# yjtang249/MIPSFusion

Measured on AMD Instinct MI355X. Metric: rays*samples/s per GPU, full optimisation iteration (fwd + bwd + pose+map Adam), 4096 rays x 64 samples, 640x480 RGB-D, higher is better.
Workload: dtype f32; decoder products as 3 x bf16 pieces of each fp32 operand, 6 bf16 MFMAs per product, fp32 accumulate; 1 GPU; BASELINE config 2: FastCaMo-synth apartment_2, 1 active submap per GPU, 4096 rays x 64 samples, hash grid 2^19 x 16 x 2, 620x460 synthetic RGB-D; rays=4096, samples_per_ray=64, hash_size=19, parallelism=single gpu

## Files before the change

### include/mipsf_compact.h

```cpp
#ifndef MIPSF_COMPACT_H
#define MIPSF_COMPACT_H

#include "mipsf.h"

#ifdef __cplusplus
extern "C" {
#endif

#define MIPSF_LIVE_HEADER 16u
#define MIPSF_LIVE_PAD 0xffffffffu
int mipsf_decoder_live_compact(const float* dout, uint32_t M, uint32_t* live_list, float* dfeat, float* dx, int feat_layout,
                               void* stream);

int mipsf_hashgrid_dx_from_jac_list(const float* jac, const float* dout, float* dx, const uint32_t* live_list, uint32_t M,
                                    const mipsf_grid_meta* meta_host, int layout, void* stream);

int mipsf_gather_pose_place_fwd_masked(const float* db, uint64_t n_rows, const int64_t* idx, const float* fixed_poses,
                                       const float* rot, const float* trans, uint32_t F, uint32_t K, const int64_t* owner,
                                       const float* noise, const float* z_uniform, const float* z_near_offsets,
                                       const float* z_near_nodepth, const mipsf_render_cfg* cfg_host, float* d_cam, float* rgb,
                                       float* depth, float* z_vals, float* xn, uint32_t* counts, uint32_t* wants_dx, uint32_t N,
                                       void* stream);
int mipsf_hashgrid_fwd_masked(const float* x, const float* params, float* out, float* jac, const uint32_t* ray_mask, uint32_t S,
                              uint32_t M, const mipsf_grid_meta* meta_host, int layout, void* stream);
int mipsf_hashgrid_dx_from_jac_masked(const float* jac, const float* dout, float* dx, const uint32_t* tile_live,
                                      const uint32_t* live_list, const uint32_t* ray_mask, uint32_t S, uint32_t M,
                                      const mipsf_grid_meta* meta_host, int layout, void* stream);

#ifdef __cplusplus
}
#endif
#endif
```

### mipsfusion_amd/_lib.py

```python
from __future__ import annotations

import ctypes as C
import os
from typing import Optional

import torch

_HERE = os.path.dirname(os.path.abspath(__file__))
LIB_PATH = os.environ.get("MIPSF_LIB") or os.path.join(_HERE, "libmipsf_hip.so")
MAX_LEVELS = 32
FEAT_AOS, FEAT_LEVEL_MAJOR = 0, 1
PREC = {"f32": 0, "f16x3": 1, "f16": 2, "bf16x3": 3, "bf16x6": 4}


class GridMeta(C.Structure):
    _fields_ = [("n_levels", C.c_uint32), ("n_features", C.c_uint32), ("log2_hashmap_size", C.c_uint32),
                ("base_resolution", C.c_uint32), ("per_level_scale", C.c_float),
                ("log2_per_level_scale", C.c_float), ("n_params", C.c_uint32),
                ("offsets", C.c_uint32 * (MAX_LEVELS + 1)), ("resolutions", C.c_uint32 * MAX_LEVELS),
                ("scales", C.c_float * MAX_LEVELS)]


class DecoderWeights(C.Structure):
    _fields_ = [(n, C.c_void_p) for n in ("w_pts0", "b_pts0", "w_pts2", "b_pts2", "w_rgb0", "b_rgb0",
# ... 65 lines not shown


class AdamTensors(C.Structure):
    _fields_ = [("count", C.c_uint32), ("param", C.c_void_p * ADAM_MAX_TENSORS), ("grad", C.c_void_p * ADAM_MAX_TENSORS),
                ("exp_avg", C.c_void_p * ADAM_MAX_TENSORS), ("exp_avg_sq", C.c_void_p * ADAM_MAX_TENSORS),
                ("numel", C.c_uint64 * ADAM_MAX_TENSORS)]


ADAM_MAX_GROUPS = 8
ADAM_SMALL_MAX_NUMEL = 16384


class AdamSmall(C.Structure):
    _fields_ = [("n_groups", C.c_uint32), ("n_tensors", C.c_uint32),
                ("step_dev", C.c_void_p * ADAM_MAX_GROUPS), ("hyper_dev", C.c_void_p * ADAM_MAX_GROUPS),
                ("lr", C.c_float * ADAM_MAX_GROUPS), ("beta1", C.c_float * ADAM_MAX_GROUPS),
                ("beta2", C.c_float * ADAM_MAX_GROUPS), ("eps", C.c_float * ADAM_MAX_GROUPS),
                ("weight_decay", C.c_float * ADAM_MAX_GROUPS),
                ("param", C.c_void_p * ADAM_MAX_TENSORS), ("grad", C.c_void_p * ADAM_MAX_TENSORS),
                ("exp_avg", C.c_void_p * ADAM_MAX_TENSORS), ("exp_avg_sq", C.c_void_p * ADAM_MAX_TENSORS),
                ("numel", C.c_uint32 * ADAM_MAX_TENSORS), ("group_of", C.c_uint32 * ADAM_MAX_TENSORS)]


_P = C.c_void_p
_U32, _U64, _I, _F, _D = C.c_uint32, C.c_uint64, C.c_int, C.c_float, C.c_double

SIGNATURES = {
    "mipsf_last_error": (C.c_char_p, []),
    "mipsf_abi_version": (_I, []),
    "mipsf_device_cu_count": (_I, []),
    "mipsf_buffer_size": (_U64, [_I, _U32, _U32, _U32, C.POINTER(GridMeta)]),
    "mipsf_hashgrid_meta_init": (_I, [C.POINTER(GridMeta), _U32, _U32, _U32, _U32, _D]),
    "mipsf_hashgrid_fwd": (_I, [_P, _P, _P, _P, _U32, C.POINTER(GridMeta), _I, _P]),
    "mipsf_hashgrid_dx_from_jac": (_I, [_P, _P, _P, _P, _U32, C.POINTER(GridMeta), _I, _P]),
    "mipsf_hashgrid_bwd": (_I, [C.POINTER(HashgridBwdArgs), _P]),
    "mipsf_hashgrid_route": (_I, [_P, _P, _U32, C.POINTER(GridMeta), _P]),    "mipsf_hashgrid_indices": (_I, [_P, _P, _U32, C.POINTER(GridMeta), _P]),
    "mipsf_freq_fwd": (_I, [_P, _P, _U32, _U32, _U32, _P]),
    "mipsf_freq_bwd": (_I, [_P, _P, _P, _U32, _U32, _U32, _P]),
    "mipsf_decoder_pack": (_I, [C.POINTER(DecoderWeights), _P, _P]),
    "mipsf_decoder_pack_host": (_I, [C.POINTER(DecoderWeights), _P]),
    "mipsf_decoder_fwd": (_I, [_P, _P, _I, _P, _P, _I, _P, _P, _U32, _P]),
    "mipsf_decoder_fwd_sdf": (_I, [_P, _P, _I, _P, _P, _I, _P, _U32, _P]),
    "mipsf_decoder_bwd": (_I, [_P, _P, _I, _P, _P, _I, _P, _P, _P, _P, _P, _P, C.POINTER(DecoderGrads), _P, _P,
                               _U32, _P]),
    "mipsf_decoder_bwd_chain": (_I, [_P, _I, _P, _I, _P, _P, _P, _P, _P, _P, _P, _U32, _P]),
    "mipsf_decoder_wgrad": (_I, [_P, _I, _P, _P, _I, _P, _P, C.POINTER(DecoderGrads), _P, _I, _U32, _P]),
    "mipsf_decoder_pack16": (_I, [C.POINTER(DecoderWeights), _P, _I, _P]),
    "mipsf_decoder_fwd16": (_I, [C.POINTER(DecoderFwd16Args), _P]),
    "mipsf_decoder_bwd_chain16": (_I, [C.POINTER(DecoderChain16Args), _P]),
    "mipsf_decoder_wgrad16": (_I, [C.POINTER(DecoderWgrad16Args), _P]),
    "mipsf_sample_rays": (_I, [_P, _P, _P, _P, _P, _P, _P, C.POINTER(RenderCfg), _P, _P, _P, _U32, _P]),
    "mipsf_normalise_points": (_I, [_P, C.POINTER(RenderCfg), _P, _U32, _P]),
    "mipsf_render_fwd": (_I, [C.POINTER(RenderFwdArgs), _P]),
    "mipsf_loss_finalize_sums": (_I, [_P, C.POINTER(RenderCfg), _U32, _U32, _P, _P, _P, _P]),
    "mipsf_render_bwd": (_I, [C.POINTER(RenderBwdArgs), _P]),
    "mipsf_gather_pose_place_fwd": (_I, [_P, _U64, _P, _P, _P, _P, _U32, _U32, _P, _P, _P, _P, _P, C.POINTER(RenderCfg), _P, _P,
                                         _P, _P, _P, _P, _U32, _P]),
    "mipsf_place_pose_bwd": (_I, [_P, _P, C.POINTER(RenderCfg), _P, _U32, _U32, _P, _P, _P, _P, _P, _U32, _U32, _I, _P]),
    "mipsf_rays_bwd": (_I, [_P, _P, C.POINTER(RenderCfg), _P, _P, _U32, _U32, _P]),
    "mipsf_normalise_bwd": (_I, [_P, C.POINTER(RenderCfg), _P, _U32, _P]),
    "mipsf_pose_rays_fwd": (_I, [_P, _U64, _P, _P, _P, _P, _U32, _U32, _P, _P, _P, _P, _P, _P, _U32, _P]),
    "mipsf_pose_handover": (_I, [_P, _I, _P, _P, _P]),
    "mipsf_pose_rays_bwd": (_I, [_P, _P, _P, _U32, _U32, _P, _P, _P, _P, _P, _U32, _I, _P]),
    "mipsf_adam_step": (_I, [_P, _P, _P, _P, _U64, _F, _F, _F, _F, _F, _U32, _P, _I, _P]),
    "mipsf_adam_advance_n": (_I, [_P, _P, _P, _P, _P, _U32, _P]),
    "mipsf_adam_step_multi": (_I, [C.POINTER(AdamTensors), _F, _F, _F, _F, _F, _U32, _P, _I, _P]),
    "mipsf_adam_step_small": (_I, [C.POINTER(AdamSmall), _I, _P]),
    "mipsf_adam_step_all": (_I, [C.POINTER(AdamSmall), _I, _P, _P]),
    "mipsf_ro_fitness": (_I, [_P, _U32, _P, _F, _P, _U32, _U32, _P]),
    "mipsf_ro_fitness_sdf": (_I, [_P, _P, _F, _P, _U32, _U32, _I, _P]),
    "mipsf_ro_particles": (_I, [_P, _P, _P, _P, C.POINTER(RenderCfg), _P, _P, _U32, _U32, _I, _P]),
    "mipsf_ro_update": (_I, [_P, _P, _P, _F, _F, _U32, _P]),
    "mipsf_gather_rays": (_I, [_P, _U64, _P, _U32, _P, _P, _P, _P, _P]),
}


SIZE_MCUBES_OFFSET_WORDS, SIZE_MCUBES_WELD_SLOTS, SIZE_MCUBES_WELD_WORDS = 20, 21, 22
MCUBES_BLOCK_CELLS = 4096
McubesArgs = _args("McubesArgs", [("X", _CU), ("Y", _CU), ("Z", _CU), ("isovalue", C.c_float), ("truncation", C.c_float),
                                  ("volume", _VP), ("cases", _VP), ("block_offsets", _VP), ("soup", _VP), ("cell_ids", _VP),
                                  ("capacity_tris", _CU)])
McubesWeldArgs = _args("McubesWeldArgs", [("T", _CU), ("soup", _VP), ("scratch", _VP), ("vertices", _VP), ("faces", _VP),
                                          ("counts", _VP), ("max_rounds", _CU)])
COMPACT_SIGNATURES = {
    "mipsf_decoder_live_compact": (_I, [_P, _U32, _P, _P, _P, _I, _P]),
    "mipsf_hashgrid_dx_from_jac_list": (_I, [_P, _P, _P, _P, _U32, C.POINTER(GridMeta), _I, _P]),
    "mipsf_gather_pose_place_fwd_masked": (_I, [_P, _U64, _P, _P, _P, _P, _U32, _U32, _P, _P, _P, _P, _P, C.POINTER(RenderCfg),
                                                _P, _P, _P, _P, _P, _P, _P, _U32, _P]),
    "mipsf_hashgrid_fwd_masked": (_I, [_P, _P, _P, _P, _P, _U32, _U32, C.POINTER(GridMeta), _I, _P]),
    "mipsf_hashgrid_dx_from_jac_masked": (_I, [_P, _P, _P, _P, _P, _P, _U32, _U32, C.POINTER(GridMeta), _I, _P]),
}

MESH_SIGNATURES = {
    "mipsf_mcubes_count": (_I, [C.POINTER(McubesArgs), _P]),
    "mipsf_mcubes_emit": (_I, [C.POINTER(McubesArgs), _P]),
    "mipsf_mcubes_weld": (_I, [C.POINTER(McubesWeldArgs), _P]),
}


FUSE_KF_FLOATS = 16
FUSE_IN_BOX, FUSE_SEEN = 1, 2


class FusePoints(C.Structure):
    _fields_ = [("points", _VP), ("ticks", _VP * 3), ("dims", _CU * 3), ("lo", _CU * 3), ("size", _CU * 3), ("first", _CU), ("n", _CU)]


class FuseCamera(C.Structure):
    _fields_ = [("fx", C.c_float), ("fy", C.c_float), ("cx", C.c_float), ("cy", C.c_float), ("W", C.c_float), ("H", C.c_float),
                ("edge", C.c_float), ("k", _CU), ("keyframes", _VP)]


FuseVisibilityArgs = _args("FuseVisibilityArgs", [("pts", FusePoints), ("cam", FuseCamera), ("seen", _VP)])
FuseLocalArgs = _args("FuseLocalArgs", [("pts", FusePoints), ("w2l", C.c_float * 12), ("sub", C.c_double * 3), ("div", C.c_double * 3),
                                        ("out", _VP)])
FuseAccumulateArgs = _args("FuseAccumulateArgs", [("pts", FusePoints), ("cam", FuseCamera), ("rows", _VP), ("n_rows", _CU),
                                                  ("channels", _CU), ("sigmoid", _CU), ("values", _VP), ("entropy", _VP),
                                                  ("value_stride", _CU), ("entropy_stride", _CU), ("use_obb", _CU),
                                                  ("obb_centre", C.c_double * 3), ("obb_axes", C.c_double * 9),
                                                  ("obb_half", C.c_double * 3), ("centroid", C.c_float * 3), ("sigma", C.c_float),
                                                  ("gauss_k", C.c_float), ("num", _VP), ("den", _VP), ("flags", _VP)])
FuseFinalizeArgs = _args("FuseFinalizeArgs", [("n", _CU), ("channels", _CU), ("num", _VP), ("den", _VP), ("flags", _VP), ("out", _VP),
                                              ("volume", _VP)])
FuseLabelArgs = _args("FuseLabelArgs", [("F", _CU), ("E", _CU), ("pairs", _VP), ("labels", _VP), ("counts", _VP), ("max_rounds", _CU),
                                        ("resume", _CU)])
FUSE_SIGNATURES = {
    "mipsf_fuse_visibility": (_I, [C.POINTER(FuseVisibilityArgs), _P]),
    "mipsf_fuse_local_points": (_I, [C.POINTER(FuseLocalArgs), _P]),
    "mipsf_fuse_accumulate": (_I, [C.POINTER(FuseAccumulateArgs), _P]),
    "mipsf_fuse_finalize": (_I, [C.POINTER(FuseFinalizeArgs), _P]),
    "mipsf_fuse_label_components": (_I, [C.POINTER(FuseLabelArgs), _P]),
}


ICP_KNN = 30
ICP_RESULT_DOUBLES = 20
ICP_MAX_POINTS, ICP_MAX_CELLS = 1 << 27, 1 << 26
ICP_WS_CLOUD, ICP_WS_GRID, ICP_WS_REGISTER = 1, 2, 3
IcpCloudArgs = _args("IcpCloudArgs", [("n", _CU), ("k", _CU), ("rows_per_owner", _CU), ("rows", _VP), ("owner", _VP), ("poses", _VP),
                                      ("points", _VP), ("count", _VP), ("workspace", _VP)])
IcpBinArgs = _args("IcpBinArgs", [("n", _CU), ("max_cells", _CU), ("points", _VP), ("min_edge", C.c_double), ("grid", _VP)])
IcpNearestArgs = _args("IcpNearestArgs", [("n_source", _CU), ("n_target", _CU), ("max_cells", _CU), ("source", _VP), ("grid", _VP),
                                          ("max_dist", C.c_double), ("partner", _VP), ("d2", _VP)])
IcpNormalsArgs = _args("IcpNormalsArgs", [("n", _CU), ("max_cells", _CU), ("points", _VP), ("grid", _VP), ("normals", _VP),
                                          ("neighbours", _VP)])
IcpRegisterArgs = _args("IcpRegisterArgs", [("n_source", _CU), ("n_target", _CU), ("max_cells", _CU), ("max_iteration", _CU),
                                            ("source", _VP), ("grid", _VP), ("target_normals", _VP), ("max_dist", C.c_double),
                                            ("relative_fitness", C.c_double), ("relative_rmse", C.c_double), ("result", _VP),
                                            ("partner", _VP), ("workspace", _VP)])
ICP_SIGNATURES = {
    "mipsf_icp_workspace_bytes": (_U64, [_I, _U32, _U32]),
    "mipsf_icp_cloud": (_I, [C.POINTER(IcpCloudArgs), _P]),
    "mipsf_icp_bin": (_I, [C.POINTER(IcpBinArgs), _P]),
    "mipsf_icp_nearest": (_I, [C.POINTER(IcpNearestArgs), _P]),
    "mipsf_icp_normals": (_I, [C.POINTER(IcpNormalsArgs), _P]),
    "mipsf_icp_register": (_I, [C.POINTER(IcpRegisterArgs), _P]),
}


POSEGRAPH_MAX_NODES, POSEGRAPH_MAX_EDGES, POSEGRAPH_LDS_NODES, POSEGRAPH_RESULT_DOUBLES = 64, 1024, 20, 8
POSEGRAPH_FACTORISATION_FAILED, POSEGRAPH_NAN_QUALITY, POSEGRAPH_BAD_EDGE = 1, 2, 4
PosegraphArgs = _args("PosegraphArgs", [("n_nodes", _CU), ("n_edges", _CU), ("input_f64", _CU), ("anchors", _VP), ("edges", _VP),
                                        ("observations", _VP), ("weights", _VP), ("steps", _CU), ("patience", _CU),
                                        ("max_rejects", _CU), ("reserved", _CU), ("decreasing", C.c_double), ("radius", C.c_double),
                                        ("min_diag", C.c_double), ("anchors_out", _VP), ("anchors_out32", _VP), ("result", _VP),
                                        ("workspace", _VP)])
POSEGRAPH_SIGNATURES = {
# ... 355 lines not shown
```

### mipsfusion_amd/csrc/decoder.hip

```cpp
#include "decoder_dev.h"
#include "launch.h"

namespace mipsf {
using namespace dl;


template <bool PE_INTERNAL, int LAYOUT, bool SAVE, bool SDF_ONLY = false>
__device__ __forceinline__ void decoder_fwd_tile(const float* tail, const float4* img1,
                                                 const float4* img2, const float4* img3,
                                                 const float* __restrict__ feat, const float* __restrict__ x,
                                                 const float* __restrict__ embed_pos, float* __restrict__ out,
                                                 float* __restrict__ saved, uint32_t M, int pin, int64_t tile,
                                                 int lane) {
    const int j = lane & 31, h = lane >> 5;
    const uint32_t s_raw = (uint32_t)(tile * 32 + j);
    const bool live = s_raw < M;
    const uint32_t s = live ? s_raw : M - 1;
    const uint32_t lane16 = 16u * (uint32_t)lane;
    const srd_t sv = make_srd(SAVE ? saved + (size_t)tile * ACT_TILE_FLOATS : saved, SAVE ? ACT_TILE_FLOATS * 4 : 0);

    float ev[E_SLOTS];
    load_e<PE_INTERNAL>(x, embed_pos, s, h, ev);

    f32x16 H1[4];
    load_bias(tail, 0, h, H1);
    mfma_layer<RT_F1, T_F1>(img1, lane, H1,
                            [&](int t) { return t < E_SLOTS ? ev[t] : 0.0f; });
#pragma unroll
    for (int rt = 0; rt < 4; ++rt)
#pragma unroll
        for (int r = 0; r < 16; ++r) H1[rt][r] = fmaxf(H1[rt][r], 0.0f);

    uint32_t m1[2] = {0u, 0u};
    if (SAVE) relu_masks(H1, m1);

    constexpr int RT2 = SDF_ONLY ? 2 : RT_F2;
    f32x16 H2[RT2];
    load_bias(tail, 1, h, H2);
    mfma_layer<RT2, T_F2>(img2, lane, H2,
                          [&](int t) { return H1[t >> 4][t & 15]; },
                          [&](int t4) { if constexpr (SAVE) { if (pin == 0) buf_store_act_piece(sv, lane16, 0, H1, t4); } });

    float rgb[3] = {0.f, 0.f, 0.f};
    if constexpr (!SDF_ONLY) {
        float pr[3];
        const float4* trgb = reinterpret_cast<const float4*>(tail) + h * TRGB_SLOTS;
        f32x2 p01 = {0.f, 0.f};
        float p2 = 0.f;
#pragma unroll
        for (int slot = 0; slot < 32; ++slot) {
            const float4 wv = trgb[slot];
            const float v = H2[2 + (slot >> 4)][slot & 15];
            p01 = __builtin_elementwise_fma(f32x2{wv.x, wv.y}, f32x2{v, v}, p01);
            p2 = fmaf(wv.z, v, p2);
        }
#pragma unroll
        for (int t = 0; t < E_SLOTS; ++t) {
            const float4 wv = trgb[32 + t];
            p01 = __builtin_elementwise_fma(f32x2{wv.x, wv.y}, f32x2{ev[t], ev[t]}, p01);
            p2 = fmaf(wv.z, ev[t], p2);
        }
        pr[0] = p01.x, pr[1] = p01.y, pr[2] = p2;
#pragma unroll
        for (int c = 0; c < 3; ++c) rgb[c] = (pr[c] + __shfl_xor(pr[c], 32, 64)) + tail[OFF_BSMALL - OFF_TRGB + c];
    }

    float gf[16];
    if (LAYOUT == MIPSF_FEAT_LEVEL_MAJOR && M < (1u << 24)) {
        const srd_t fs = make_srd(feat, M * 128u);
        const uint32_t voff = (2u * s + (uint32_t)h) * 4u;
#pragma unroll
        for (int u = 0; u < 16; ++u)
            gf[u] = __uint_as_float(__builtin_amdgcn_raw_buffer_load_b32(fs, voff, (uint32_t)u * M * 8u, 0));
    } else {
#pragma unroll
        for (int u = 0; u < 16; ++u) gf[u] = load_feat<LAYOUT>(feat, s, u, h, M);
    }
    f32x16 H3[4];
    load_bias(tail, 2, h, H3);
    mfma_layer<RT_F3, T_F3>(img3, lane, H3,
                            [&](int t) { return t < 32 ? H2[t >> 4][t & 15] : gf[t - 32]; },
                            [&](int t4) {
                                if constexpr (SAVE) {
// ... 617 lines not shown
        if (!tile_live) zero16(nx);
        put_act(XT, nx, 0, 4, 0, w, lane);
        put_act(YT, ny, 2, 2, 0, w, lane);
        {
            float ev[E_SLOTS];
            load_e<PE_INTERNAL>(x, embed_pos, s, h, ev);
#pragma unroll
            for (int t = 0; t < E_SLOTS; ++t) {
                const int e = eidx(t, h);
                if (e >= 0) YT[e * WG_LDW + 32 * w + j] = ev[t];
            }
        }
        {
            float* pad = YT + (51 + bhalf) * WG_LDW + brow;
#pragma unroll
            for (int i = 0; i < 7; ++i)
                if (bhalf + 2 * i < 13) pad[2 * i * WG_LDW] = (bhalf + 2 * i == 0) ? 1.0f : 0.0f;
        }
        X8[(4 * bhalf + 0) * WG_LDW + brow] = nsm.x;
        X8[(4 * bhalf + 1) * WG_LDW + brow] = nsm.y;
        X8[(4 * bhalf + 2) * WG_LDW + brow] = nsm.z;
        X8[(4 * bhalf + 3) * WG_LDW + brow] = nsm.w;
        __syncthreads();
        {
            const char* by = act_base(saved, tile, 2, 0);
            auto fetch = [&](int g) { ny[g] = act_piece(by, g, lane16); };
            if constexpr (BF16X3) wgrad_mma_bf16<2>(XT, YT, w, 0, lane, aW1, fetch);
            else wgrad_mma<2>(XT, YT, w, 0, lane, aW1, fetch);
        }
        wgrad_mma_small(X8, YT, w, lane, aRGB);
        __syncthreads();

        put_act(YT, ny, 0, 4, 0, w, lane);
        __syncthreads();
        {
            const uint32_t nb = bt + gridDim.x;
            const int nt = src_tile(nb);
            const char* bx = act_base(dact, nt, 2, 0);
            const char* by = act_base(saved, nt, 1, 0);
            const uint32_t ns = sample_of(nb);
            wgrad_mma_small(X8, YT, w, lane, aS2, [&](int g) {
                nx[g] = act_piece(bx, g, lane16);
                if (g < 8) ny[g] = act_piece(by, g, lane16);
                ngf[g] = load_feat<LAYOUT>(feat, ns, g, h, M);
            });
        }
        __syncthreads();
    }

    float* rec = partial + (size_t)blockIdx.x * (G_STRIDE + 0);
    for (int q = tid; q < G_STRIDE; q += DEC_BLOCK) rec[q] = 0.0f;
    __syncthreads();
#pragma unroll
    for (int ct = 0; ct < 3; ++ct) flush_tile(rec, G_W_SDF0, HID, N_SDF_IN, w, ct, lane, aS1[ct]);
#pragma unroll
    for (int ct = 0; ct < 4; ++ct) flush_tile(rec, G_W_PTS2, HID, HID, w, ct, lane, aW2[ct]);
#pragma unroll
    for (int ct = 0; ct < 2; ++ct) flush_tile(rec, G_W_PTS0, HID, N_E, w, ct, lane, aW1[ct]);
    {
#pragma unroll
        for (int ct = 0; ct < 2; ++ct)
#pragma unroll
            for (int r = 0; r < 4; ++r) {
                const int row = 4 * (lane >> 4) + r, col = 32 * w + 16 * ct + (lane & 15);
                if (row < N_CLASS) rec[G_W_SDF2 + row * HID + col] = aS2[ct][r];
                const int rc = col < N_E ? 64 + col : (col >= 64 ? col - 64 : -1);
                if (row >= 5 && row < 8 && rc >= 0) rec[G_W_RGB0 + (row - 5) * N_RGB_IN + rc] = aRGB[ct][r];
                if (col == N_E && row < N_CLASS) rec[G_B_SDF2 + row] = aRGB[ct][r];
                if (col == N_E && row >= 5 && row < 8) rec[G_B_RGB0 + row - 5] = aRGB[ct][r];
            }
    }
    {
        const int jj = lane & 31, hh = lane >> 5;
        if (jj == N_E - 32) {
#pragma unroll
            for (int r = 0; r < 16; ++r) rec[G_B_PTS0 + 32 * w + rowmap(r, hh)] = aW1[1][r];
        }
    }
    atomicAdd(&rec[G_B_SDF0 + brow], db3);
    atomicAdd(&rec[G_B_PTS2 + brow], db2);
}


struct GradPtrs {
    float* p[10];
};

constexpr int WG_REDUCE_SLICES = 8;
__global__ __launch_bounds__(256) void decoder_wgrad_reduce_kernel(const float* __restrict__ partial, uint32_t nrec,
                                                                   GradPtrs g) {
    const int q = blockIdx.x * blockDim.x + threadIdx.x;
    if (q >= G_TOTAL) return;
    float a0 = 0.f, a1 = 0.f, a2 = 0.f, a3 = 0.f;
    uint32_t b = blockIdx.y;
    for (; b + 3 * WG_REDUCE_SLICES < nrec; b += 4 * WG_REDUCE_SLICES) {
        a0 += partial[(size_t)b * G_STRIDE + q];
        a1 += partial[(size_t)(b + WG_REDUCE_SLICES) * G_STRIDE + q];
        a2 += partial[(size_t)(b + 2 * WG_REDUCE_SLICES) * G_STRIDE + q];
        a3 += partial[(size_t)(b + 3 * WG_REDUCE_SLICES) * G_STRIDE + q];
    }
    for (; b < nrec; b += WG_REDUCE_SLICES) a0 += partial[(size_t)b * G_STRIDE + q];
    const float a = (a0 + a1) + (a2 + a3);
    const int bounds[11] = {G_W_PTS0, G_B_PTS0, G_W_PTS2, G_B_PTS2, G_W_RGB0, G_B_RGB0,
                            G_W_SDF0, G_B_SDF0, G_W_SDF2, G_B_SDF2, G_TOTAL};
#pragma unroll
    for (int k = 0; k < 10; ++k)
        if (q >= bounds[k] && q < bounds[k + 1]) unsafeAtomicAdd(&g.p[k][q - bounds[k]], a);
}

__global__ __launch_bounds__(256) void decoder_pack_kernel(W w, float* __restrict__ packed) {
    const int idx = blockIdx.x * blockDim.x + threadIdx.x;
    if (idx < PACKED_FLOATS) packed[idx] = packed_value(w, idx);
}

static W to_w(const mipsf_decoder_weights& s) {
    W w;
    w.w_pts0 = s.w_pts0, w.b_pts0 = s.b_pts0, w.w_pts2 = s.w_pts2, w.b_pts2 = s.b_pts2, w.w_rgb0 = s.w_rgb0;
    w.b_rgb0 = s.b_rgb0, w.w_sdf0 = s.w_sdf0, w.b_sdf0 = s.b_sdf0, w.w_sdf2 = s.w_sdf2, w.b_sdf2 = s.b_sdf2;
    return w;
}

constexpr uint32_t WG_MAX_BLOCKS = 256;

__global__ __launch_bounds__(256) void decoder_wgrad_reduce_fixed_kernel(const float* __restrict__ partial, uint32_t nrec,
                                                                         GradPtrs g) {
    const int q = blockIdx.x * blockDim.x + threadIdx.x;
    if (q >= G_TOTAL) return;
    float a = 0.f;
    for (uint32_t b = 0; b < nrec; ++b) a += partial[(size_t)b * G_STRIDE + q];
    const int bounds[11] = {G_W_PTS0, G_B_PTS0, G_W_PTS2, G_B_PTS2, G_W_RGB0, G_B_RGB0,
                            G_W_SDF0, G_B_SDF0, G_W_SDF2, G_B_SDF2, G_TOTAL};
#pragma unroll
    for (int k = 0; k < 10; ++k)
        if (q >= bounds[k] && q < bounds[k + 1]) {
            float* p = &g.p[k][q - bounds[k]];
            *p = *p + a;
        }
}

int wgrad_reduce_launch(const float* partial, uint32_t nrec, const mipsf_decoder_grads* grads, hipStream_t s, bool fixed_order) {
    if (fixed_order) {
        GradPtrs g;
        g.p[0] = grads->w_pts0, g.p[1] = grads->b_pts0, g.p[2] = grads->w_pts2, g.p[3] = grads->b_pts2;
        g.p[4] = grads->w_rgb0, g.p[5] = grads->b_rgb0, g.p[6] = grads->w_sdf0, g.p[7] = grads->b_sdf0;
        g.p[8] = grads->w_sdf2, g.p[9] = grads->b_sdf2;
        for (int k = 0; k < 10; ++k) MIPSF_REQUIRE(g.p[k] != nullptr, "null gradient pointer %d", k);
        hipLaunchKernelGGL(decoder_wgrad_reduce_fixed_kernel, dim3((G_TOTAL + 255) / 256), dim3(256), 0, s, partial, nrec, g);
        return check_launch("decoder_wgrad_reduce_fixed");
    }
    return wgrad_reduce_launch(partial, nrec, grads, s);
}

int wgrad_reduce_launch(const float* partial, uint32_t nrec, const mipsf_decoder_grads* grads, hipStream_t s) {
    GradPtrs g;
    g.p[0] = grads->w_pts0, g.p[1] = grads->b_pts0, g.p[2] = grads->w_pts2, g.p[3] = grads->b_pts2;
    g.p[4] = grads->w_rgb0, g.p[5] = grads->b_rgb0, g.p[6] = grads->w_sdf0, g.p[7] = grads->b_sdf0;
    g.p[8] = grads->w_sdf2, g.p[9] = grads->b_sdf2;
    for (int k = 0; k < 10; ++k) MIPSF_REQUIRE(g.p[k] != nullptr, "null gradient pointer %d", k);
    hipLaunchKernelGGL(decoder_wgrad_reduce_kernel, dim3((G_TOTAL + 255) / 256, WG_REDUCE_SLICES), dim3(256), 0, s, partial,
                       nrec, g);
    return check_launch("decoder_wgrad_reduce");
}

static inline uint64_t n_wave_tiles(uint32_t M) { return ((uint64_t)M + 31) / 32; }
static inline uint64_t n_block_tiles(uint32_t M) { return ((uint64_t)M + 127) / 128; }

uint64_t decoder_packed_floats() { return (uint64_t)PACKED_FLOATS; }
uint64_t decoder_saved_floats(uint32_t M) { return n_block_tiles(M) * 4 * (ACT_TILE_FLOATS + MASK_TILE_WORDS); }
uint64_t decoder_dact_floats(uint32_t M) { return n_block_tiles(M) * 4 * ACT_TILE_FLOATS + n_block_tiles(M) * 128 * 8; }
uint64_t decoder_wgrad_partial_floats() { return (uint64_t)WG_MAX_BLOCKS * G_STRIDE; }

}

using namespace mipsf;

extern "C" {

int mipsf_decoder_pack(const mipsf_decoder_weights* w, float* packed, void* stream) {
    MIPSF_REQUIRE(w && packed, "null pointer");
    hipLaunchKernelGGL(decoder_pack_kernel, dim3((PACKED_FLOATS + 255) / 256), dim3(256), 0, (hipStream_t)stream,
                       to_w(*w), packed);
    return check_launch("decoder_pack");
}

int mipsf_decoder_pack_host(const mipsf_decoder_weights* w, float* packed_host) {
    MIPSF_REQUIRE(w && packed_host, "null pointer");
    const W ww = to_w(*w);
    for (int idx = 0; idx < PACKED_FLOATS; ++idx) packed_host[idx] = packed_value(ww, idx);
    return 0;
}

static int decoder_fwd_launch(const float* packed, const float* feat, int feat_layout, const float* x,
                              const float* embed_pos, int pe_mode, float* out, float* saved, bool sdf_only, uint32_t M,
                              void* stream) {
    if (M == 0) return 0;
    MIPSF_REQUIRE(packed && feat && x && out, "null pointer");
    MIPSF_REQUIRE(pe_mode == 0 || embed_pos, "pe_mode 1 needs embed_pos");
    MIPSF_REQUIRE(feat_layout == MIPSF_FEAT_AOS || feat_layout == MIPSF_FEAT_LEVEL_MAJOR, "bad layout");
    const uint32_t n_tiles = (uint32_t)n_wave_tiles(M);
    const uint32_t blocks = (n_tiles + 3) / 4;
    hipStream_t s = (hipStream_t)stream;
    const int cus = device_cus();
    if (cus <= 0) return 3;
    const bool persistent = n_tiles >= (uint32_t)cus * 8u * MIPSF_FWD_LDS_MIN_ROUNDS;
    return with_bool(pe_mode == 0, [&](auto PE) { return with_layout(feat_layout, [&](auto LAY) {
        auto arm = [&](auto SAVE, auto SDF) {
            if (persistent) {
                constexpr auto kern = decoder_fwd_lds_kernel<PE.value, LAY.value, SAVE.value, SDF.value>;
                if (!grant_lds<kern>(FWD_LDS_BYTES)) return lds_refused(FWD_LDS_BYTES);
                hipLaunchKernelGGL(kern, dim3(cus), dim3(FWD_LDS_BLOCK), FWD_LDS_BYTES, s, packed, feat, x, embed_pos, out, saved,
                                   M, 0, n_tiles);
            } else {
                hipLaunchKernelGGL((decoder_fwd_kernel<PE.value, LAY.value, SAVE.value, SDF.value>), dim3(blocks), dim3(DEC_BLOCK), 0,
                                   s, packed, feat, x, embed_pos, out, saved, M, 0);
            }
            return check_launch("decoder_fwd");
        };
        return sdf_only ? arm(no, yes) : saved != nullptr ? arm(yes, no) : arm(no, no);
    }); });
}

int mipsf_decoder_fwd(const float* packed, const float* feat, int feat_layout, const float* x,
                      const float* embed_pos, int pe_mode, float* out, float* saved, uint32_t M, void* stream) {
    return decoder_fwd_launch(packed, feat, feat_layout, x, embed_pos, pe_mode, out, saved, false, M, stream);
}

int mipsf_decoder_fwd_sdf(const float* packed, const float* feat, int feat_layout, const float* x,
                          const float* embed_pos, int pe_mode, float* sdf, uint32_t M, void* stream) {
    return decoder_fwd_launch(packed, feat, feat_layout, x, embed_pos, pe_mode, sdf, nullptr, true, M, stream);
}

int mipsf_decoder_bwd_chain(const float* packed, int feat_layout, const float* x, int pe_mode, const float* out,
                            const float* dout, const float* saved, float* dfeat, float* dx, float* dembed_pos,
                            float* dact, uint32_t M, void* stream) {
    if (M == 0) return 0;
    MIPSF_REQUIRE(packed && x && out && dout && saved && dfeat && dx && dact, "null pointer");
    MIPSF_REQUIRE(pe_mode == 0 || dembed_pos, "pe_mode 1 needs dembed_pos");
    MIPSF_REQUIRE(feat_layout == MIPSF_FEAT_AOS || feat_layout == MIPSF_FEAT_LEVEL_MAJOR, "bad layout");
    hipStream_t s = (hipStream_t)stream;
    const uint32_t blocks = (uint32_t)((n_wave_tiles(M) + 3) / 4);
    float* dsmall = dact + n_block_tiles(M) * 4 * ACT_TILE_FLOATS;
    return with_bool(pe_mode == 0, [&](auto PE) { return with_layout(feat_layout, [&](auto LAY) {
        hipLaunchKernelGGL((decoder_bwd_lds_kernel<PE.value, LAY.value>), dim3(blocks), dim3(DEC_BLOCK), 0, s, packed, x, out, dout,
                           saved, dfeat, dx, dembed_pos, dact, dsmall, M, MIPSF_PIN_ARG);
        return check_launch("decoder_bwd_chain");
    }); });
}

static int decoder_wgrad_launch(const float* feat, int feat_layout, const float* x, const float* embed_pos, int pe_mode,
                               const float* saved, const float* dact, const mipsf_decoder_grads* grads, float* partial,
                               bool bf16x3, uint32_t M, void* stream);
int mipsf_decoder_wgrad(const float* feat, int feat_layout, const float* x, const float* embed_pos, int pe_mode,
                        const float* saved, const float* dact, const mipsf_decoder_grads* grads, float* partial,
                        int precision, uint32_t M, void* stream) {
    MIPSF_REQUIRE(precision == MIPSF_PREC_F32 || precision == MIPSF_PREC_BF16X3, "precision must be f32 or bf16x3");
    return decoder_wgrad_launch(feat, feat_layout, x, embed_pos, pe_mode, saved, dact, grads, partial,
                                precision == MIPSF_PREC_BF16X3, M, stream);
}
static int decoder_wgrad_launch(const float* feat, int feat_layout, const float* x, const float* embed_pos, int pe_mode,
                               const float* saved, const float* dact, const mipsf_decoder_grads* grads, float* partial,
                               bool bf16x3, uint32_t M, void* stream) {
    if (M == 0) return 0;
    MIPSF_REQUIRE(feat && x && saved && dact && partial && grads, "null pointer");
    MIPSF_REQUIRE(pe_mode == 0 || embed_pos, "pe_mode 1 needs embed_pos");
    MIPSF_REQUIRE(feat_layout == MIPSF_FEAT_AOS || feat_layout == MIPSF_FEAT_LEVEL_MAJOR, "bad layout");
    hipStream_t s = (hipStream_t)stream;
    const uint32_t n_bt = (uint32_t)n_block_tiles(M);
    const float* dsmall = dact + n_block_tiles(M) * 4 * ACT_TILE_FLOATS;
    GradPtrs g;
    g.p[0] = grads->w_pts0, g.p[1] = grads->b_pts0, g.p[2] = grads->w_pts2, g.p[3] = grads->b_pts2;
    g.p[4] = grads->w_rgb0, g.p[5] = grads->b_rgb0, g.p[6] = grads->w_sdf0, g.p[7] = grads->b_sdf0;
    g.p[8] = grads->w_sdf2, g.p[9] = grads->b_sdf2;
    for (int k = 0; k < 10; ++k) MIPSF_REQUIRE(g.p[k] != nullptr, "null gradient pointer %d", k);
    const int cus = device_cus();
    if (cus <= 0) return 3;
    uint32_t wg_blocks = n_bt < (uint32_t)cus ? n_bt : (uint32_t)cus;
    if (wg_blocks > WG_MAX_BLOCKS) wg_blocks = WG_MAX_BLOCKS;
    const int rc = with_bool(pe_mode == 0, [&](auto PE) { return with_layout(feat_layout, [&](auto LAY) {
        return with_bool(bf16x3, [&](auto BF) {
            constexpr auto kern = decoder_wgrad_kernel<PE.value, LAY.value, BF.value>;
            if (!grant_lds<kern>(WG_LDS_BYTES)) return lds_refused(WG_LDS_BYTES);
            hipLaunchKernelGGL(kern, dim3(wg_blocks), dim3(DEC_BLOCK), WG_LDS_BYTES, s, feat, x, embed_pos, saved, dact, dsmall,
                               partial, M, n_bt);
            return check_launch("decoder_wgrad");
        });
    }); });
    if (rc) return rc;
    hipLaunchKernelGGL(decoder_wgrad_reduce_kernel, dim3((G_TOTAL + 255) / 256, WG_REDUCE_SLICES), dim3(256), 0, s, partial, wg_blocks, g);
    return check_launch("decoder_wgrad_reduce");
}

int mipsf_decoder_bwd(const float* packed, const float* feat, int feat_layout, const float* x,
                      const float* embed_pos, int pe_mode, const float* out, const float* dout,
                      const float* saved, float* dfeat, float* dx, float* dembed_pos,
                      const mipsf_decoder_grads* grads, float* dact, float* partial, uint32_t M, void* stream) {
    if (int e = mipsf_decoder_bwd_chain(packed, feat_layout, x, pe_mode, out, dout, saved, dfeat, dx, dembed_pos, dact,
                                        M, stream))
        return e;
    return mipsf_decoder_wgrad(feat, feat_layout, x, embed_pos, pe_mode, saved, dact, grads, partial, MIPSF_PREC_F32, M, stream);
}

}
```

### mipsfusion_amd/csrc/hashgrid.hip

```cpp
#include "common.h"
#include "launch.h"
#include "decoder_layout.h"

namespace mipsf {

constexpr uint32_t P1 = 2654435761u;
constexpr uint32_t P2 = 805459861u;
constexpr int HG_BLOCK = 256;

struct Cell {
    uint32_t c[3];
    float f[3];
};

__device__ __forceinline__ Cell locate(const float* __restrict__ x, uint32_t i, float scale) {
    Cell r;
#pragma unroll
    for (int d = 0; d < 3; ++d) {
        const float pos = fmaf(scale, x[3 * (size_t)i + d], 0.5f);
        const float fl = floorf(pos);
        r.c[d] = (uint32_t)(int)fl;
        r.f[d] = pos - fl;
    }
    return r;
}

template <int MODE>
__device__ __forceinline__ uint32_t corner_index(uint32_t cx, uint32_t cy, uint32_t cz, uint32_t res,
                                                 uint32_t size) {
    if (MODE == 0) {
        uint32_t idx = cx + cy * res + cz * res * res;
        if (idx >= size) {
            idx -= size;
            if (idx >= size) idx %= size;
        }
        return idx;
    }
    const uint32_t h = cx ^ (cy * P1) ^ (cz * P2);
    return MODE == 1 ? (h & (size - 1u)) : (h % size);
}

__host__ __device__ inline bool level_is_hashed(uint32_t res, uint32_t size) {
    uint64_t stride = 1;
    for (int d = 0; d < 3; ++d) {
        if (stride > size) break;
        stride *= res;
        stride &= 0xFFFFFFFFull;
    }
    return size < stride;
}

__device__ __forceinline__ int decode_level(uint32_t n_levels, uint32_t nchunk, uint32_t& chunk) {
    const uint32_t b = blockIdx.x;
    const uint32_t xcd = b & 7u;
    const uint32_t j = b >> 3;
    const uint32_t slot = j / nchunk;
    chunk = j - slot * nchunk;
    const uint32_t nslots = (n_levels + 7u) / 8u;
    return (int)(xcd + 8u * (nslots - 1u - slot));
}

template <int MODE>
__device__ __forceinline__ void corner_indices_m(const Cell& cell, uint32_t res, uint32_t size, uint32_t idx[8]) {
#pragma unroll
    for (int c = 0; c < 8; ++c) {
        idx[c] = corner_index<MODE>(cell.c[0] + (c & 1), cell.c[1] + ((c >> 1) & 1), cell.c[2] + ((c >> 2) & 1),
                                    res, size);
    }
}

__device__ __forceinline__ int level_mode(uint32_t res, uint32_t size) {
    if (!level_is_hashed(res, size)) return 0;
    return (size & (size - 1u)) == 0u ? 1 : 2;
}

__device__ __forceinline__ void corner_indices(int mode, const Cell& cell, uint32_t res, uint32_t size,
                                               uint32_t idx[8]) {
    if (mode == 0) corner_indices_m<0>(cell, res, size, idx);
    else if (mode == 1) corner_indices_m<1>(cell, res, size, idx);
    else corner_indices_m<2>(cell, res, size, idx);
}

__device__ __forceinline__ void corner_weights(const Cell& cell, float w[8]) {
#pragma unroll
    for (int c = 0; c < 8; ++c) {
// ... 182 lines not shown
    if (i < n) ws[i] = 0u;
}

__device__ __forceinline__ uint32_t ranked_add(uint32_t* cnt, uint32_t s, bool active, bool aggregate) {
    if (!aggregate) return active ? atomicAdd(&cnt[s], 1u) : 0u;
    const uint32_t lane = threadIdx.x & 63u;
    uint32_t rank = 0;
    unsigned long long todo = __ballot(active);
    while (todo) {
        const int leader = __ffsll((long long)todo) - 1;
        const uint32_t s0 = (uint32_t)__shfl((int)s, leader, 64);
        const unsigned long long m = __ballot(active && s == s0);
        uint32_t b = 0;
        if ((int)lane == leader) b = atomicAdd(&cnt[s0], (uint32_t)__popcll(m));
        b = (uint32_t)__shfl((int)b, leader, 64);
        if (active && s == s0) rank = b + (uint32_t)__popcll(m & ((1ull << lane) - 1ull));
        todo &= ~m;
    }
    return rank;
}

__device__ __forceinline__ void route_groups_general(int mode, const Cell& cell, uint32_t res, uint32_t size,
                                                     uint32_t shift, uint32_t (&s)[8], uint32_t (&m)[8]) {
    uint32_t idx[8];
    corner_indices(mode, cell, res, size, idx);
#pragma unroll
    for (int c = 0; c < 8; ++c) s[c] = idx[c] >> shift;
#pragma unroll
    for (int c = 0; c < 8; ++c) {
        bool first = true;
        uint32_t mm = 0;
#pragma unroll
        for (int k = 0; k < 8; ++k) {
            if (k < c) first = first && (s[k] != s[c]);
            mm |= (s[k] == s[c]) ? (1u << k) : 0u;
        }
        m[c] = first ? mm : 0u;
    }
}

__device__ __forceinline__ bool route_groups_dense(const Cell& cell, uint32_t res, uint32_t size, uint32_t shift,
                                                   uint32_t (&s)[8], uint32_t (&m)[8]) {
    uint32_t idx[8];
    corner_indices_m<0>(cell, res, size, idx);
    const uint32_t lo = idx[0] >> shift, hi = idx[7] >> shift;
    uint32_t m_lo = 0, m_hi = 0;
#pragma unroll
    for (int c = 0; c < 8; ++c) {
        const uint32_t q = idx[c] >> shift;
        m_lo |= (q == lo) ? (1u << c) : 0u;
        m_hi |= (q == hi) ? (1u << c) : 0u;
    }
    s[0] = lo, m[0] = m_lo;
    s[1] = hi, m[1] = hi != lo ? m_hi : 0u;
    return (m_lo | m_hi) == 0xffu;
}

__device__ __forceinline__ bool route_groups_hashed_pow2(const Cell& cell, uint32_t size, uint32_t shift,
                                                         uint32_t (&s)[8], uint32_t (&m)[8]) {
#pragma unroll
    for (int p = 0; p < 4; ++p) {
        const uint32_t cy = cell.c[1] + (p & 1), cz = cell.c[2] + (p >> 1);
        s[p] = ((cell.c[0] ^ (cy * P1) ^ (cz * P2)) & (size - 1u)) >> shift;
        m[p] = 3u << (2 * p);
    }
#pragma unroll
    for (int p = 1; p < 4; ++p)
#pragma unroll
        for (int q = 0; q < p; ++q) {
            const bool same = m[p] != 0u && m[q] != 0u && s[q] == s[p];
            m[q] |= same ? m[p] : 0u;
            m[p] = same ? 0u : m[p];
        }
    return cell.c[0] < (1u << shift) - 1u;
}

#ifndef MIPSF_RT_LEVELS
#define MIPSF_RT_LEVELS 1
#endif
constexpr uint32_t RT_LEVELS = MIPSF_RT_LEVELS;
__host__ __device__ inline uint32_t route_groups(uint32_t n_levels) { return (n_levels + RT_LEVELS - 1) / RT_LEVELS; }

template <int LAYOUT>
__global__ __launch_bounds__(RT_BLOCK) void scatter_route_kernel(const float* __restrict__ x,
                                                                const float* __restrict__ dout, uint32_t M, GridLevels g,
                                                                ScatterPlan plan, uint32_t* __restrict__ ws,
                                                                uint32_t* __restrict__ cw) {
    __shared__ uint32_t cnt[SC_MAX_NS];
    __shared__ uint32_t base[SC_MAX_NS];
#ifndef MIPSF_SC_STAGE
#define MIPSF_SC_STAGE 1
#endif
#ifndef MIPSF_SC_STAGE_CAP
#define MIPSF_SC_STAGE_CAP (10 * RT_BLOCK)
#endif
    constexpr uint32_t STAGE_CAP = MIPSF_SC_STAGE_CAP;
    __shared__ uint32_t lstart[SC_MAX_NS];
    __shared__ uint32_t stage[MIPSF_SC_STAGE ? STAGE_CAP : 1];
    const uint32_t n_groups = route_groups(plan.n_levels);
    const uint32_t group = blockIdx.x % n_groups;
    const uint32_t chunk = blockIdx.x / n_groups;
#ifndef MIPSF_SC_AGG_MAX
#define MIPSF_SC_AGG_MAX 1
#endif
#ifndef MIPSF_SC_ROUTE_FAST
#define MIPSF_SC_ROUTE_FAST 1
#endif
#ifdef MIPSF_RT_TRACE
    unsigned long long tr_t[10];
    unsigned long long tr_acc[9] = {0ull, 0ull, 0ull, 0ull, 0ull, 0ull, 0ull, 0ull, 0ull};
#define RT_MARK(k) do { __builtin_amdgcn_sched_barrier(0); tr_t[k] = __builtin_amdgcn_s_memtime(); __builtin_amdgcn_sched_barrier(0); } while (0)
#else
#define RT_MARK(k) do { } while (0)
#endif
    RT_MARK(0);
    const uint32_t s0 = chunk * (RT_BLOCK * SC_ROUTE_UNR);
    __shared__ uint32_t live_list[RT_BLOCK * SC_ROUTE_UNR];
    __shared__ uint32_t wave_base[(RT_BLOCK / 64) * SC_ROUTE_UNR + 1];
    {
        const uint32_t wave = threadIdx.x >> 6, lane = threadIdx.x & 63u;
        unsigned long long alive[SC_ROUTE_UNR];
        float2 gy[SC_ROUTE_UNR][RT_LEVELS];
        if (dout != nullptr) {
#pragma unroll
            for (uint32_t u = 0; u < SC_ROUTE_UNR; ++u) {
                const uint32_t i = s0 + u * RT_BLOCK + threadIdx.x;
#pragma unroll
                for (uint32_t k = 0; k < RT_LEVELS; ++k) {
                    const uint32_t level = group + k * n_groups;
                    gy[u][k] = (i < M && level < plan.n_levels)
                                   ? *reinterpret_cast<const float2*>(dout + feat_index<LAYOUT>(i, level, M, plan.n_levels))
                                   : make_float2(0.f, 0.f);
                }
            }
        }
#pragma unroll
        for (uint32_t u = 0; u < SC_ROUTE_UNR; ++u) {
            const uint32_t i = s0 + u * RT_BLOCK + threadIdx.x;
            bool live = i < M;
            if (live && dout != nullptr) {
                live = false;
#pragma unroll
                for (uint32_t k = 0; k < RT_LEVELS; ++k) live = live || !(gy[u][k].x == 0.0f && gy[u][k].y == 0.0f);
            }
            alive[u] = __ballot(live);
            if (lane == 0) wave_base[1 + u * (RT_BLOCK / 64) + wave] = (uint32_t)__popcll(alive[u]);
        }
        RT_MARK(1);
        __syncthreads();
        static_assert((RT_BLOCK / 64) * SC_ROUTE_UNR <= 64, "one wave scans the (round, wave) counts");
        if (threadIdx.x < 64) {
            uint32_t v = threadIdx.x < (RT_BLOCK / 64) * SC_ROUTE_UNR ? wave_base[1 + threadIdx.x] : 0u;
#pragma unroll
            for (int d = 1; d < 64; d <<= 1) {
                const uint32_t o = (uint32_t)__shfl_up((int)v, d, 64);
                v += (int)threadIdx.x >= d ? o : 0u;
            }
            if (threadIdx.x < (RT_BLOCK / 64) * SC_ROUTE_UNR) wave_base[1 + threadIdx.x] = v;
            if (threadIdx.x == 0) wave_base[0] = 0u;
        }
        __syncthreads();
#pragma unroll
        for (uint32_t u = 0; u < SC_ROUTE_UNR; ++u)
            if (alive[u] >> lane & 1ull)
                live_list[wave_base[u * (RT_BLOCK / 64) + wave] + (uint32_t)__popcll(alive[u] & ((1ull << lane) - 1ull))] =
                    s0 + u * RT_BLOCK + threadIdx.x;
        __syncthreads();
    }
    RT_MARK(2);
    const uint32_t n_live = wave_base[(RT_BLOCK / 64) * SC_ROUTE_UNR];
    uint32_t mine[SC_ROUTE_UNR];
    float xr[SC_ROUTE_UNR][3];
#pragma unroll
    for (uint32_t u = 0; u < SC_ROUTE_UNR; ++u) {
        const uint32_t c = u * RT_BLOCK + threadIdx.x;
        const uint32_t i = c < n_live ? live_list[c] : 0u;
        mine[u] = i;
#pragma unroll
        for (int d = 0; d < 3; ++d) xr[u][d] = x[3 * (size_t)i + d];
    }
    const bool masked = M <= SC_MASKED_MAX_M;
    uint32_t* rec = ws + plan.w_records;
#ifdef MIPSF_RT_TRACE
    tr_acc[0] = tr_t[1] - tr_t[0], tr_acc[1] = tr_t[2] - tr_t[1];
// ... 49 lines not shown
        if (wide) {
#pragma unroll
            for (int q = 4; q < 8; ++q) r[q] = ranked_add(cnt, s[q], m[q] != 0u, aggregate);
        }
#pragma unroll
        for (int q = 0; q < 4; ++q) {
            sp[u][q] = s[2 * q] | (s[2 * q + 1] << 16);
            rp[u][q] = r[2 * q] | (r[2 * q + 1] << 16);
        }
        mp[u][0] = m[0] | (m[1] << 8) | (m[2] << 16) | (m[3] << 24);
        mp[u][1] = m[4] | (m[5] << 8) | (m[6] << 16) | (m[7] << 24);
    }
    RT_MARK(3);
    __syncthreads();
    RT_MARK(4);
    for (uint32_t q = threadIdx.x; q < ns; q += RT_BLOCK)
        base[q] = cnt[q] ? atomicAdd(&cw[plan.w_count + bin0 + q], cnt[q]) : 0u;
    if (MIPSF_SC_STAGE && threadIdx.x < 64) {
        constexpr uint32_t PER = SC_MAX_NS / 64;
        uint32_t c[PER], sum = 0;
#pragma unroll
        for (uint32_t q2 = 0; q2 < PER; ++q2) {
            const uint32_t q = threadIdx.x * PER + q2;
            c[q2] = q < ns ? cnt[q] : 0u;
            sum += c[q2];
        }
        uint32_t incl = sum;
#pragma unroll
        for (int d = 1; d < 64; d <<= 1) {
            const uint32_t v = (uint32_t)__shfl_up((int)incl, d, 64);
            incl += (int)threadIdx.x >= d ? v : 0u;
        }
        uint32_t run = incl - sum;
#pragma unroll
        for (uint32_t q2 = 0; q2 < PER; ++q2) {
            const uint32_t q = threadIdx.x * PER + q2;
            if (q < ns) lstart[q] = run;
            run += c[q2];
        }
    }
    RT_MARK(5);
    __syncthreads();
    RT_MARK(6);
#pragma unroll
    for (uint32_t u = 0; u < SC_ROUTE_UNR; ++u) {
        const uint32_t i = mine[u];
#pragma unroll
        for (int q = 0; q < 8; ++q) {
            if (q == 4 && !__any(mp[u][1] != 0u)) break;
            const uint32_t m = (mp[u][q >> 2] >> (8 * (q & 3))) & 0xffu;
            if (m) {
                const uint32_t sl = (sp[u][q >> 1] >> (16 * (q & 1))) & 0xffffu;
                const uint32_t rk = (rp[u][q >> 1] >> (16 * (q & 1))) & 0xffffu;
                if (MIPSF_SC_STAGE) {
                    const uint32_t p = lstart[sl] + rk;
                    if (p < STAGE_CAP) {
                        stage[p] = masked ? (i | (m << 24)) : i;
                        continue;
                    }
                }
                rec[(size_t)(bin0 + sl) * M + base[sl] + rk] = masked ? (i | (m << 24)) : i;
            }
        }
    }
    RT_MARK(7);
    if (MIPSF_SC_STAGE) {
        __syncthreads();
        RT_MARK(8);
        const uint32_t wave = threadIdx.x >> 6, lane = threadIdx.x & 63u;
        for (uint32_t q = wave; q < ns; q += RT_BLOCK / 64) {
            const uint32_t n = cnt[q], src = lstart[q];
            uint32_t* dstp = rec + (size_t)(bin0 + q) * M + base[q];
            for (uint32_t p = lane; p < n && src + p < STAGE_CAP; p += 64) dstp[p] = stage[src + p];
        }
    }
#ifdef MIPSF_RT_TRACE
    RT_MARK(9);
    for (int q = 2; q < 9; ++q) tr_acc[q] += tr_t[q + 1] - tr_t[q];
    ++tr_levels;
#endif
    }
#ifdef MIPSF_RT_TRACE
    if ((threadIdx.x & 63u) == 0u) {
        unsigned long long* tr = reinterpret_cast<unsigned long long*>(ws + plan.w_end + 64) + (size_t)(blockIdx.x * (RT_BLOCK / 64) + (threadIdx.x >> 6)) * 10;
        for (int q = 0; q < 9; ++q) tr[q] = tr_acc[q];
        tr[9] = (unsigned long long)(group | (tr_levels << 8));
    }
#endif
}
__device__ __forceinline__ uint32_t part_of(const ScatterPlan& plan, uint32_t bin) {
    return bin < plan.dense_bins ? SC_PART_DENSE : SC_PART;
}

#ifndef MIPSF_SC_PUBLISH_WT
#define MIPSF_SC_PUBLISH_WT 1
#endif

template <bool AGENT>
__device__ __forceinline__ float2 fold_entry(const float2* p2, uint32_t parts, float2 cur) {
    float2 a = make_float2(0.f, 0.f);
    for (uint32_t q = 0; q < parts; q += 8) {
        float2 v[8];
#pragma unroll
        for (uint32_t k = 0; k < 8; ++k) {
            v[k] = make_float2(0.f, 0.f);
            if (q + k < parts) {
                if (AGENT) {
                    const unsigned long long u = __hip_atomic_load(
                        reinterpret_cast<const unsigned long long*>(p2 + (size_t)(q + k) * SC_MAX_SLICE), __ATOMIC_RELAXED,
                        __HIP_MEMORY_SCOPE_AGENT);
                    v[k] = make_float2(__uint_as_float((uint32_t)u), __uint_as_float((uint32_t)(u >> 32)));
                } else {
                    v[k] = p2[(size_t)(q + k) * SC_MAX_SLICE];
                }
            }
        }
#pragma unroll
        for (uint32_t k = 0; k < 8; ++k) a.x += v[k].x, a.y += v[k].y;
    }
    cur.x += a.x, cur.y += a.y;
    return cur;
}

template <int LAYOUT>
__device__ __forceinline__ void scatter_item(const float* __restrict__ x, const float* __restrict__ dout,
                                             float* __restrict__ dparams, uint32_t M, const GridLevels& g,
                                             const ScatterPlan& plan, uint32_t* __restrict__ ws, uint32_t* __restrict__ cw,
                                             uint32_t* sh_flag, double* __restrict__ acc,
                                             const uint4 desc, const uint32_t item_index) {
    const uint32_t item = desc.x;
    const uint32_t sc_plane1 = plan.max_slice;
    (void)sc_plane1;
    const uint32_t bin = item & 0xffffu, part = item >> 16;
    const bool single = desc.z == 1u;
    uint32_t level = 0;
    while (level + 1 < plan.n_levels && bin >= plan.bin0[level + 1]) ++level;
    const uint32_t slice = bin - plan.bin0[level];
    const uint32_t off = g.offsets[level];
    const uint32_t size = g.offsets[level + 1] - off;
    const uint32_t se = plan.slice_entries[level];
    const uint32_t begin = slice * se;
    const uint32_t count = begin + se <= size ? se : size - begin;
    const uint32_t res = g.res[level];
    const float scale = g.scale[level];
    const uint32_t n_rec_bin = desc.y;
    const uint32_t r0 = part * part_of(plan, bin);
    const uint32_t n_rec = n_rec_bin - r0 < part_of(plan, bin) ? n_rec_bin - r0 : part_of(plan, bin);
    const uint32_t* __restrict__ rec = ws + plan.w_records + (size_t)bin * M + r0;

    {
#if MIPSF_SC_PLANAR
        for (uint32_t e = threadIdx.x; e < count; e += SC_BLOCK) acc[SC_ACC0(e)] = 0.0, acc[SC_ACC1(e)] = 0.0;
#else
        double2* z = reinterpret_cast<double2*>(acc);
        for (uint32_t e = threadIdx.x; e < count; e += SC_BLOCK) z[e] = make_double2(0.0, 0.0);
#endif
    }
    float2* dst = reinterpret_cast<float2*>(dparams) + off + begin;
    constexpr uint32_t FL = SC_MAX_SLICE / SC_BLOCK;
    float2 cur[FL];
    if (single && !plan.fresh) {
#pragma unroll
        for (uint32_t k = 0; k < FL; ++k) {
            const uint32_t e = threadIdx.x + k * SC_BLOCK;
            cur[k] = e < count ? dst[e] : make_float2(0.f, 0.f);
        }
    }
    __syncthreads();

    const int mode = level_mode(res, size);
    const bool masked = M <= SC_MASKED_MAX_M;
// ... 315 lines not shown
        __syncthreads();
        if (t == 0) {
            const uint64_t tr_t1 = wall_clock64();
            uint32_t* tr = ws + plan.w_end + 64 + 8 * (size_t)i;
            tr[0] = i, tr[1] = desc.x, tr[2] = desc.y, tr[3] = (uint32_t)tr_t0, tr[4] = (uint32_t)tr_t1;
            tr[5] = __builtin_amdgcn_s_getreg((31 << 11) | 20), tr[6] = blockIdx.x, tr[7] = desc.z;
            if (i == 0) ws[plan.w_end + 63] = total;
        }
#endif
    }
    __syncthreads();
    if (t == 0) {
        if (__hip_atomic_fetch_add(&cw[plan.w_nitems + 2], 1u, __ATOMIC_RELAXED, __HIP_MEMORY_SCOPE_AGENT) == gridDim.x - 1) {
            __hip_atomic_store(&cw[plan.w_nitems], 0u, __ATOMIC_RELAXED, __HIP_MEMORY_SCOPE_AGENT);
            __hip_atomic_store(&cw[plan.w_nitems + 1], 0u, __ATOMIC_RELAXED, __HIP_MEMORY_SCOPE_AGENT);
            __hip_atomic_store(&cw[plan.w_nitems + 2], 0u, __ATOMIC_RELAXED, __HIP_MEMORY_SCOPE_AGENT);
        }
    }
}

__global__ __launch_bounds__(256) void hashgrid_scatter_reduce_kernel(float* __restrict__ dparams, GridLevels g,
                                                                      ScatterPlan plan, const uint32_t* __restrict__ ws,
                                                                      const uint32_t* __restrict__ cw) {
    const uint32_t bin = blockIdx.x;
    const uint32_t parts = cw[plan.w_parts + bin];
    if (parts <= 1) return;
    uint32_t level = 0;
    while (level + 1 < plan.n_levels && bin >= plan.bin0[level + 1]) ++level;
    const uint32_t size = g.offsets[level + 1] - g.offsets[level];
    const uint32_t se = plan.slice_entries[level];
    const uint32_t begin = (bin - plan.bin0[level]) * se;
    const uint32_t count = begin + se <= size ? se : size - begin;
    const uint32_t e = blockIdx.y * 256 + threadIdx.x;
    if (e >= count) return;
    const float2* p2 = reinterpret_cast<const float2*>(reinterpret_cast<const float*>(ws) + plan.w_partial) +
                       (size_t)cw[plan.w_first + bin] * SC_MAX_SLICE + e;
    float2* d = reinterpret_cast<float2*>(dparams) + g.offsets[level] + begin + e;
    *d = fold_entry<false>(p2, parts, plan.fresh ? make_float2(0.f, 0.f) : *d);
}

template <int LAYOUT>
MIPSF_SINGLE_FP32 __global__ __launch_bounds__(HG_BLOCK) void hashgrid_dx_kernel(const float* __restrict__ x,
                                                               const float2* __restrict__ table,
                                                               const float* __restrict__ dout,
                                                               float* __restrict__ dxl, uint32_t M, GridLevels g,
                                                               uint32_t nchunk) {
    uint32_t chunk;
    const int level = decode_level(g.n_levels, nchunk, chunk);
    if (level >= (int)g.n_levels) return;
    const uint32_t i = chunk * HG_BLOCK + threadIdx.x;
    if (i >= M) return;
    const uint32_t off = g.offsets[level];
    const uint32_t size = g.offsets[level + 1] - off;
    const uint32_t res = g.res[level];
    const float scale = g.scale[level];
    const Cell cell = locate(x, i, scale);
    uint32_t idx[8];
    corner_indices(level_mode(res, size), cell, res, size, idx);
    const float2 gy = *reinterpret_cast<const float2*>(dout + feat_index<LAYOUT>(i, level, M, g.n_levels));
    const float2* lvl = table + off;
    float2 v[8];
#pragma unroll
    for (int c = 0; c < 8; ++c) v[c] = lvl[idx[c]];
    float gx[3];
#pragma unroll
    for (int d = 0; d < 3; ++d) {
        float s0, s1;
        level_jacobian(cell, v, scale, d, s0, s1);
        gx[d] = s0 * gy.x + s1 * gy.y;
    }
    float* o = dxl + ((size_t)level * M + i) * 3;
    o[0] = gx[0], o[1] = gx[1], o[2] = gx[2];
}

__global__ __launch_bounds__(256) void hashgrid_dx_reduce_kernel(const float* __restrict__ dxl, float* __restrict__ dx,
                                                                 uint64_t n3, uint32_t L) {
    const uint64_t t = (uint64_t)blockIdx.x * blockDim.x + threadIdx.x;
    if (t >= n3) return;
    float a = 0.f;
    for (uint32_t l = 0; l < L; ++l) a += dxl[(uint64_t)l * n3 + t];
    dx[t] += a;
}

template <int LAYOUT>
MIPSF_SINGLE_FP32 __global__ __launch_bounds__(256) void hashgrid_dx_jac_kernel(const float* __restrict__ jac,
                                                              const float* __restrict__ dout, float* __restrict__ dx,
                                                              uint32_t M, uint32_t L,
                                                              const uint32_t* __restrict__ tiles,
                                                              const uint32_t* __restrict__ live_list,
                                                              const uint32_t* __restrict__ ray_mask, uint32_t S) {
    uint32_t i = blockIdx.x * blockDim.x + threadIdx.x;
    if (live_list != nullptr) {
        if (i >= M || i >= live_list[0]) return;
        i = live_list[MIPSF_LIVE_HEADER + i];
    }
    if (tiles != nullptr) {
        const uint32_t k = i >> 5, cap = mipsf::dl::tl_cap((M + 31u) / 32u);
        uint32_t q = 0, first = 0, total = 0;
#pragma unroll
        for (uint32_t j = 0; j < 8; ++j) {
            const uint32_t n = tiles[64 * j + 32];
            if (k >= total && n != 0u) q = j, first = total;
            total += n;
        }
        if (k >= total) return;
        i = tiles[mipsf::dl::TL_HEADER + q * cap + (k - first)] * 32u + (i & 31u);
    }
    if (i >= M) return;
    if (!ray_wants_dx(ray_mask, S, i)) {
        dx[3 * (size_t)i] = 0.f, dx[3 * (size_t)i + 1] = 0.f, dx[3 * (size_t)i + 2] = 0.f;
        return;
    }
    float a[3] = {0.f, 0.f, 0.f};
    for (uint32_t l = 0; l < L; ++l) {
        const float2* j2 = reinterpret_cast<const float2*>(jac) + (size_t)l * 3 * M + i;
        const float2 gy = *reinterpret_cast<const float2*>(dout + feat_index<LAYOUT>(i, l, M, L));
#pragma unroll
        for (int d = 0; d < 3; ++d) {
            const float2 j = j2[(size_t)d * M];
            a[d] += j.x * gy.x + j.y * gy.y;
        }
    }
    dx[3 * (size_t)i] += a[0], dx[3 * (size_t)i + 1] += a[1], dx[3 * (size_t)i + 2] += a[2];
}

__global__ __launch_bounds__(HG_BLOCK) void hashgrid_indices_kernel(const float* __restrict__ x,
                                                                    uint32_t* __restrict__ out, uint32_t M,
                                                                    GridLevels g, uint32_t nchunk) {
    uint32_t chunk;
    const int level = decode_level(g.n_levels, nchunk, chunk);
    if (level >= (int)g.n_levels) return;
    const uint32_t i = chunk * HG_BLOCK + threadIdx.x;
    if (i >= M) return;
    const uint32_t size = g.offsets[level + 1] - g.offsets[level];
    const uint32_t res = g.res[level];
    const Cell cell = locate(x, i, g.scale[level]);
    uint32_t idx[8];
    corner_indices(level_mode(res, size), cell, res, size, idx);
#pragma unroll
    for (int c = 0; c < 8; ++c) out[((size_t)i * g.n_levels + level) * 8 + c] = idx[c];
}

static int to_levels(const mipsf_grid_meta* m, GridLevels& g) {
    MIPSF_REQUIRE(m != nullptr, "meta is null");
    MIPSF_REQUIRE(m->n_features == 2, "only n_features_per_level == 2 is built");
    MIPSF_REQUIRE(m->n_levels >= 1 && m->n_levels <= MIPSF_MAX_LEVELS, "bad n_levels");
    g.n_levels = m->n_levels;
    for (uint32_t l = 0; l <= m->n_levels; ++l) g.offsets[l] = m->offsets[l];
    for (uint32_t l = 0; l < m->n_levels; ++l) {
        g.res[l] = m->resolutions[l];
        g.scale[l] = m->scales[l];
    }
    return 0;
}

static inline uint32_t grid_blocks(uint32_t M, uint32_t L, uint32_t& nchunk) {
    nchunk = (M + HG_BLOCK - 1) / HG_BLOCK;
    return 8u * ((L + 7u) / 8u) * nchunk;
}

constexpr uint32_t DET_BLOCK = 256;
constexpr uint32_t DET_PER_THREAD = 16;
constexpr uint32_t DET_TILE = DET_BLOCK * DET_PER_THREAD;
constexpr uint32_t DET_PIECE = MIPSF_HG_DET_PIECE;
static_assert((DET_PIECE & (DET_PIECE - 1u)) == 0u, "the piece length is a power of two");

template <int LAYOUT>
__global__ __launch_bounds__(DET_BLOCK) void det_emit_kernel(const float* __restrict__ x, const float* __restrict__ dout,
                                                             uint32_t* __restrict__ keys, uint32_t M, GridLevels g,
                                                             uint32_t dead) {
    const uint32_t level = blockIdx.y;
    const uint32_t i = blockIdx.x * DET_BLOCK + threadIdx.x;
    if (i >= M) return;
    const float2 gy = *reinterpret_cast<const float2*>(dout + feat_index<LAYOUT>(i, level, M, g.n_levels));
    uint32_t k[8];
    if (gy.x == 0.f && gy.y == 0.f) {
#pragma unroll
        for (int c = 0; c < 8; ++c) k[c] = dead;
    } else {
        const uint32_t off = g.offsets[level];
        const uint32_t size = g.offsets[level + 1] - off;
        const uint32_t res = g.res[level];
        const Cell cell = locate(x, i, g.scale[level]);
        corner_indices(level_mode(res, size), cell, res, size, k);
#pragma unroll
        for (int c = 0; c < 8; ++c) k[c] += off;
    }
    uint4* dst = reinterpret_cast<uint4*>(keys + ((size_t)level * M + i) * 8);
    dst[0] = make_uint4(k[0], k[1], k[2], k[3]);
    dst[1] = make_uint4(k[4], k[5], k[6], k[7]);
}

__device__ __forceinline__ uint32_t det_block_scan(uint32_t v, uint32_t* s) {
    s[threadIdx.x] = v;
    __syncthreads();
    for (uint32_t o = 1; o < DET_BLOCK; o <<= 1) {
        const uint32_t t = threadIdx.x >= o ? s[threadIdx.x - o] : 0u;
        __syncthreads();
        s[threadIdx.x] += t;
        __syncthreads();
    }
    return s[threadIdx.x];
}

__global__ __launch_bounds__(DET_BLOCK) void det_count_kernel(const uint32_t* __restrict__ keys, uint32_t* __restrict__ cnt,
                                                              uint32_t n, uint32_t nb, uint32_t shift) {
// ... 299 lines not shown
    GridLevels g;
    if (int rc = to_levels(meta, g)) return rc;
    if (M == 0) return 0;
    MIPSF_REQUIRE(jac && dout && dx, "null pointer");
    MIPSF_REQUIRE(layout == MIPSF_FEAT_AOS || layout == MIPSF_FEAT_LEVEL_MAJOR, "bad layout %d", layout);
    MIPSF_REQUIRE(!(tile_live && live_list), "tile_live and live_list are alternatives");
    if (int rc = check_ray_mask(ray_mask, S, M)) return rc;
    hipStream_t s = (hipStream_t)stream;
    return with_layout(layout, [&](auto LAY) {
        hipLaunchKernelGGL(hashgrid_dx_jac_kernel<LAY.value>, dim3((M + 255) / 256), dim3(256), 0, s, jac, dout, dx, M, g.n_levels,
                           tile_live, live_list, ray_mask, S);
        return check_launch("hashgrid_dx_from_jac");
    });
}
int mipsf_hashgrid_dx_from_jac_masked(const float* jac, const float* dout, float* dx, const uint32_t* tile_live,
                                      const uint32_t* live_list, const uint32_t* ray_mask, uint32_t S, uint32_t M,
                                      const mipsf_grid_meta* meta, int layout, void* stream) {
    return dx_from_jac(jac, dout, dx, tile_live, live_list, M, meta, layout, stream, ray_mask, S);
}
int mipsf_hashgrid_dx_from_jac(const float* jac, const float* dout, float* dx, const uint32_t* tile_live, uint32_t M,
                               const mipsf_grid_meta* meta, int layout, void* stream) {
    return dx_from_jac(jac, dout, dx, tile_live, nullptr, M, meta, layout, stream);
}
int mipsf_hashgrid_dx_from_jac_list(const float* jac, const float* dout, float* dx, const uint32_t* live_list, uint32_t M,
                                    const mipsf_grid_meta* meta, int layout, void* stream) {
    MIPSF_REQUIRE(live_list != nullptr, "null live_list");
    return dx_from_jac(jac, dout, dx, nullptr, live_list, M, meta, layout, stream);
}

}
namespace mipsf {
uint64_t hashgrid_bwd_scratch_floats(const mipsf_grid_meta* meta, uint32_t M, int need_dx) {
    GridLevels g;
    if (to_levels(meta, g)) return 0;
    const ScatterPlan p = make_plan(g, M);
#ifdef MIPSF_SC_TRACE
    return p.w_end + 64 + 8ull * p.max_items + 64;
#endif
#ifdef MIPSF_RT_TRACE
    return p.w_end + 64 + 20ull * (RT_BLOCK / 64) * (route_groups(g.n_levels) * ((M + RT_BLOCK * SC_ROUTE_UNR - 1) / (RT_BLOCK * SC_ROUTE_UNR))) + 64;
#endif
    return p.w_end + (need_dx ? (uint64_t)g.n_levels * M * 3 : 0) + 64;
}
uint64_t hashgrid_counter_words(const mipsf_grid_meta* meta) {
    GridLevels g;
    if (to_levels(meta, g)) return 0;
    return make_plan(g, 1).w_items;
}
}
extern "C" {


#ifdef MIPSF_SC_TRACE
uint64_t mipsf_hashgrid_trace_words(const mipsf_grid_meta* meta, uint32_t M, uint32_t* n_rows, uint32_t* bin0) {
    GridLevels g;
    if (to_levels(meta, g)) return 0;
    const ScatterPlan p = make_plan(g, M);
    *n_rows = p.max_items;
    for (uint32_t l = 0; l <= g.n_levels; ++l) bin0[l] = p.bin0[l];
    return p.w_end + 64;
}
#endif


#ifdef MIPSF_RT_TRACE
uint64_t mipsf_hashgrid_rt_trace_words(const mipsf_grid_meta* meta, uint32_t M, uint32_t* n_rows) {
    GridLevels g;
    if (to_levels(meta, g)) return 0;
    const ScatterPlan p = make_plan(g, M);
    *n_rows = (RT_BLOCK / 64) * route_groups(g.n_levels) * ((M + RT_BLOCK * SC_ROUTE_UNR - 1) / (RT_BLOCK * SC_ROUTE_UNR));
    return p.w_end + 64;
}
#endif

static int check_plan(const ScatterPlan& plan, const GridLevels& g, uint32_t M) {
    MIPSF_REQUIRE(plan.n_bins <= SC_MAX_BINS && plan.n_bins <= 0xffffu, "grid too large: %u table slices", plan.n_bins);
    for (uint32_t l = 0; l < g.n_levels; ++l)
        MIPSF_REQUIRE(plan.n_slices[l] <= SC_MAX_NS, "level %u too large: %u slices", l, plan.n_slices[l]);
    MIPSF_REQUIRE(plan.w_end < (1ull << 32), "batch too large for 32-bit scratch offsets (M = %u)", M);
    MIPSF_REQUIRE(((uint64_t)M + SC_PART_MIN - 1) / SC_PART_MIN < (1u << 16), "batch too large (M = %u)", M);
    return 0;
}

static int launch_route(const float* x, const float* dout, int layout, uint32_t* ws, uint32_t* cw, bool clear, uint32_t M,
                        const GridLevels& g, const ScatterPlan& plan, hipStream_t s) {
    if (clear) {
        const uint32_t nz = plan.w_first;
        hipLaunchKernelGGL(scatter_zero_kernel, dim3((nz + 255) / 256), dim3(256), 0, s, cw, nz);
    }
    const uint32_t rb = route_groups(g.n_levels) * ((M + RT_BLOCK * SC_ROUTE_UNR - 1) / (RT_BLOCK * SC_ROUTE_UNR));
    return with_layout(layout, [&](auto LAY) {
        hipLaunchKernelGGL(scatter_route_kernel<LAY.value>, dim3(rb), dim3(RT_BLOCK), 0, s, x, dout, M, g, plan, ws, cw);
        return check_launch("hashgrid_route");
    });
}

int mipsf_hashgrid_route(const float* x, float* scratch, uint32_t M, const mipsf_grid_meta* meta, void* stream) {
    GridLevels g;
    if (int rc = to_levels(meta, g)) return rc;
    if (M == 0) return 0;
    MIPSF_REQUIRE(x && scratch, "null pointer");
    const ScatterPlan plan = make_plan(g, M);
    if (int rc = check_plan(plan, g, M)) return rc;
    uint32_t* ws = reinterpret_cast<uint32_t*>(scratch);
    return launch_route(x, nullptr, MIPSF_FEAT_AOS, ws, ws, true, M, g, plan, (hipStream_t)stream);
}

static int hashgrid_bwd_impl(const float* x, const float* params, const float* dout, float* dparams, float* dx,
                             float* scratch, uint32_t* counters, uint32_t M, const mipsf_grid_meta* meta, int layout,
                             bool routed, void* stream, bool fresh = false) {
    GridLevels g;
    if (int rc = to_levels(meta, g)) return rc;
    if (M == 0) return 0;
    MIPSF_REQUIRE(x && params && dout && scratch, "null pointer");
    MIPSF_REQUIRE(dparams || dx, "nothing to compute: dparams and dx are both null");
    MIPSF_REQUIRE(layout == MIPSF_FEAT_AOS || layout == MIPSF_FEAT_LEVEL_MAJOR, "bad layout %d", layout);
    hipStream_t s = (hipStream_t)stream;
    ScatterPlan plan = make_plan(g, M);
    plan.fresh = fresh ? 1u : 0u;
    {
        const char* e = getenv("MIPSF_SC_FOLD_LAUNCH");
        plan.fold_launch = (e && e[0] && e[0] != '0') ? 1u : 0u;
    }
    if (int rc = check_plan(plan, g, M)) return rc;
    uint32_t* ws = reinterpret_cast<uint32_t*>(scratch);
    uint32_t* cw = counters ? counters : ws;
    float* dxl = scratch + ((plan.w_end + 15) / 16) * 16;
    if (dparams) {
        if (!routed)
            if (int e = launch_route(x, MIPSF_SC_SKIP_ZERO ? dout : nullptr, layout, ws, cw, counters == nullptr, M, g, plan, s)) return e;
        const uint32_t lds_bytes = plan.max_slice * 16 + plan.n_bins * 4;
        const int cus = device_cus();
        if (cus <= 0) return 3;
        uint32_t per_cu = (160u * 1024u) / (lds_bytes + 256u);
        per_cu = per_cu < 1u ? 1u : (per_cu > 2048u / SC_BLOCK ? 2048u / SC_BLOCK : per_cu);
        const uint32_t want = (uint32_t)cus * per_cu;
        const uint32_t blocks = plan.max_items < want ? plan.max_items : want;
        const int rc = with_layout(layout, [&](auto LAY) {
            constexpr auto kern = hashgrid_scatter_persist_kernel<LAY.value>;
            if (!grant_lds<kern>(lds_bytes)) return lds_refused(lds_bytes);
            hipLaunchKernelGGL(kern, dim3(blocks), dim3(SC_BLOCK), lds_bytes, s, x, dout, dparams, M, g, plan, ws, cw);
            return check_launch("hashgrid_scatter");
        });
        if (rc) return rc;
        if (plan.fold_launch) {
            hipLaunchKernelGGL(hashgrid_scatter_reduce_kernel, dim3(plan.n_bins, (plan.max_slice + 255) / 256), dim3(256), 0, s,
                               dparams, g, plan, ws, cw);
            if (int e = check_launch("hashgrid_scatter_reduce")) return e;
        }
    }
    if (dx) return launch_dx(x, params, dout, dxl, dx, M, g, layout, s);
    return 0;
}

int mipsf_hashgrid_bwd(const mipsf_hashgrid_bwd_args* a, void* stream) {
    MIPSF_REQUIRE(a != nullptr, "null argument block");
    MIPSF_REQUIRE(a->struct_size == sizeof(mipsf_hashgrid_bwd_args), "mipsf_hashgrid_bwd_args: struct_size %u, this library expects %u",
                  a->struct_size, (unsigned)sizeof(mipsf_hashgrid_bwd_args));
    MIPSF_REQUIRE((a->flags & ~(uint32_t)(MIPSF_HG_DPARAMS_ZERO | MIPSF_HG_ROUTED | MIPSF_HG_DETERMINISTIC)) == 0u,
                  "unknown flags 0x%x", a->flags);
    if (a->flags & MIPSF_HG_DETERMINISTIC) {
        MIPSF_REQUIRE(!(a->flags & MIPSF_HG_ROUTED), "MIPSF_HG_DETERMINISTIC with MIPSF_HG_ROUTED: the routed scratch belongs to "
                      "the fast scatter; the deterministic path takes its own scratch (MIPSF_SIZE_HASHGRID_DET_SCRATCH)");
        return hashgrid_bwd_det(a->x, a->params, a->dout, a->dparams, a->dx, a->scratch, a->M, a->meta, a->feat_layout,
                                (a->flags & MIPSF_HG_DPARAMS_ZERO) != 0u, stream);
    }
    return hashgrid_bwd_impl(a->x, a->params, a->dout, a->dparams, a->dx, a->scratch, a->counters, a->M, a->meta, a->feat_layout,
                             (a->flags & MIPSF_HG_ROUTED) != 0u, stream, (a->flags & MIPSF_HG_DPARAMS_ZERO) != 0u);
}

int mipsf_hashgrid_indices(const float* x, uint32_t* idx, uint32_t M, const mipsf_grid_meta* meta, void* stream) {
    GridLevels g;
    if (int rc = to_levels(meta, g)) return rc;
    if (M == 0) return 0;
    MIPSF_REQUIRE(x && idx, "null pointer");
    uint32_t nchunk;
    const uint32_t nb = grid_blocks(M, g.n_levels, nchunk);
    hipLaunchKernelGGL(hashgrid_indices_kernel, dim3(nb), dim3(HG_BLOCK), 0, (hipStream_t)stream, x, idx, M, g,
                       nchunk);
    return check_launch("hashgrid_indices");
}

}
```

### mipsfusion_amd/csrc/wgrad16.hip

```cpp
#include "decoder_dev.h"
#include "launch.h"

namespace mipsf {
using namespace dl;

typedef __bf16 bf8 __attribute__((ext_vector_type(8)));
typedef _Float16 h8 __attribute__((ext_vector_type(8)));
typedef float f32x8 __attribute__((ext_vector_type(8)));

struct ArF16 { typedef h8 v8; typedef _Float16 elt; static constexpr int P = 2; static constexpr bool SCALED = true; };
struct ArBF3 { typedef bf8 v8; typedef __bf16 elt; static constexpr int P = 3; static constexpr bool SCALED = false; };
struct ArBF2 { typedef bf8 v8; typedef __bf16 elt; static constexpr int P = 2; static constexpr bool SCALED = false; };
constexpr float W16_GRID_SHIFT = 4096.0f;
template <typename A> constexpr float w16_acc_unscale() { return A::SCALED ? 1.0f / (float)(1 << W16_SHIFT) : 1.0f; }
template <typename A> constexpr float w16_grid_shift() { return A::SCALED ? W16_GRID_SHIFT : 1.0f; }

__device__ __forceinline__ f32x16 mfma16(bf8 a, bf8 b, f32x16 c) { return __builtin_amdgcn_mfma_f32_32x32x16_bf16(a, b, c, 0, 0, 0); }
__device__ __forceinline__ f32x16 mfma16(h8 a, h8 b, f32x16 c) { return __builtin_amdgcn_mfma_f32_32x32x16_f16(a, b, c, 0, 0, 0); }

template <typename A, bool LAST>
__device__ __forceinline__ typename A::v8 next_plane(f32x8& r) {
    typename A::v8 pl;
    if constexpr (A::SCALED && !LAST) {
        typedef _Float16 h2_t __attribute__((ext_vector_type(2)));
// ... 1180 lines not shown
            live_start[q] = n_tiles;
            n_tiles += (uint32_t)__builtin_amdgcn_readfirstlane((int)live[64 * q + 32]);
        }
    }
    if constexpr (CP) n_tiles = (uint32_t)__builtin_amdgcn_readfirstlane((int)live_list[1]);
    const int j = lane & 31, h = lane >> 5;
    typename A::v8 I[2];
#pragma unroll
    for (int q = 0; q < 2; ++q)
#pragma unroll
        for (int u = 0; u < 8; ++u)
            I[q][u] = (j == 16 * q + 8 * (u >> 2) + 4 * h + (u & 3)) ? (typename A::elt)1.0f : (typename A::elt)0.0f;
    constexpr int W1_ENTRIES = RT_F1 * T16H_F1 * 64;
    static_assert(T16H_F1 == T16_F1, "layer 1 has no separate bias k-step");
    typedef W16XL<A> L;
    constexpr int P = A::P;
    constexpr int SCR_ENTRIES = 8 * (W16T_PLANE / 16);
    __shared__ h8 w1img[RECOMP ? P * W1_ENTRIES : 1];
    __shared__ h8 xch[RECOMP ? L::NBUF * (L::XE + L::XA + L::XB) : 1];
    __shared__ h8 gimg[RECOMP ? L::G_ENTRIES : 1];
    __shared__ h8 tscr[RECOMP ? SCR_ENTRIES : 1];
    static_assert(!RECOMP || sizeof(h8) * (P * W1_ENTRIES + L::NBUF * (L::XE + L::XA + L::XB) + L::G_ENTRIES + SCR_ENTRIES) <= 160 * 1024,
                  "the exchange form's images and hand-over buffers must fit the LDS of a CU");
    if constexpr (RECOMP) {
        const h8* img = reinterpret_cast<const h8*>(packed16 + TAIL16_FLOATS);
        const h8* ext = reinterpret_cast<const h8*>(packed16 + PACKED16_FLOATS);
        for (int q = tid; q < W1_ENTRIES; q += W16_BLOCK) {
            w1img[q] = img[OFF16H_F1 / 8 + q];
            w1img[W1_ENTRIES + q] = img[(IMG16H_HALVES + OFF16L_F1) / 8 + q];
            if constexpr (P == 3) w1img[2 * W1_ENTRIES + q] = ext[(EXT16_FWD + OFF16L_F1) / 8 + q];
        }
        const h8* bimg = img + OFF16_BWD_HALVES / 8;
        for (int q = tid; q < 4 * 64; q += W16_BLOCK) {
            gimg[q] = bimg[OFF16B_S2T / 8 + q];
            gimg[L::G_PLANE_S2T + q] = bimg[(IMG16B_HALVES + OFF16B_S2T) / 8 + q];
            if constexpr (P == 3) gimg[2 * L::G_PLANE_S2T + q] = ext[(EXT16_BWD + OFF16B_S2T) / 8 + q];
        }
        for (int q = tid; q < 2 * 64; q += W16_BLOCK) {
            gimg[L::G_RGBT + q] = bimg[OFF16B_RGBT / 8 + q];
            gimg[L::G_RGBT + L::G_PLANE_RGBT + q] = bimg[(IMG16B_HALVES + OFF16B_RGBT) / 8 + q];
            if constexpr (P == 3) gimg[L::G_RGBT + 2 * L::G_PLANE_RGBT + q] = ext[(EXT16_BWD + OFF16B_RGBT) / 8 + q];
        }
        __syncthreads();
    }
    const W16Args a = {feat, x, saved, dact, dsmall, partial + (size_t)blockIdx.x * G_STRIDE, M, n_tiles,
                       live, tl_cap(n_tiles_all),
                       {live_start[0], live_start[1], live_start[2], live_start[3], live_start[4], live_start[5],
                        live_start[6], live_start[7]},
                       RECOMP ? w1img : nullptr, RECOMP ? w1img + W1_ENTRIES : nullptr,
                       (RECOMP && lean_dact) ? gimg : nullptr,
                       reinterpret_cast<const uint2*>(saved + (((size_t)M + 127) / 128) * 4 * ACT_TILE_FLOATS),
                       CP ? live_list + MIPSF_LIVE_HEADER : nullptr, saved_bytes};
    static_assert(!CP || RECOMP, "compact mode is built into the transpose-read exchange form only");
    if constexpr (RECOMP) {
        const uint32_t xb0 = w16t_lds_addr(xch);
        const W16T<A> lx = {xb0, xb0 + 16u * L::NBUF * L::XE, xb0 + 16u * L::NBUF * (L::XE + L::XA),
                            w16t_lds_addr(tscr) + (uint32_t)w * W16T_PLANE};
        if (w < 4) w16t_role_a<LAYOUT, A, CP>(a, lx, w, lane);
        else w16t_role_b<LAYOUT, A, CP>(a, lx, I, w - 4, lane);
    } else {
        if (w < 4) w16_role_a<LAYOUT, A>(a, I, w, lane);
        else w16_role_b<LAYOUT, A>(a, I, w - 4, lane);
    }
}

}

using namespace mipsf;

#ifdef W16_TRACE
extern "C" int mipsf_w16_trace_read(unsigned long long* host, int clear) {
    if (hipMemcpyFromSymbol(host, HIP_SYMBOL(w16_trace), sizeof(unsigned long long) * 2048 * 16) != hipSuccess) return 1;
    if (clear) {
        static unsigned long long z[2048 * 16];
        if (hipMemcpyToSymbol(HIP_SYMBOL(w16_trace), z, sizeof(z)) != hipSuccess) return 1;
    }
    return 0;
}
#endif
namespace mipsf {
uint64_t decoder_tile_words(uint32_t M) { return TL_HEADER + 8ull * tl_cap((uint32_t)(((uint64_t)M + 31) / 32)); }
}

extern "C" int mipsf_decoder_wgrad16(const mipsf_decoder_wgrad16_args* a, void* stream) {
    MIPSF_REQUIRE(a != nullptr, "null argument block");
    MIPSF_REQUIRE(a->struct_size == sizeof(mipsf_decoder_wgrad16_args), "mipsf_decoder_wgrad16_args: struct_size %u, this library expects %u",
                  a->struct_size, (unsigned)sizeof(mipsf_decoder_wgrad16_args));
    const float* packed16 = a->packed16; const float* feat = a->feat; const int feat_layout = a->feat_layout; const float* x = a->x;
    const float* saved = a->saved; const float* dact = a->dact; const uint32_t* tile_live = a->tile_live;
    const mipsf_decoder_grads* grads = a->grads; float* partial = a->partial; const int arithmetic = a->arithmetic;
    const uint32_t flags = a->flags, M = a->M;
    const uint32_t* live_list = a->live_list;
    MIPSF_REQUIRE(packed16 == nullptr || a->packed16_floats == 0u || a->packed16_floats == decoder_packed16_floats(arithmetic),
                  "packed16 holds %u floats, arithmetic %d needs %u: packed for the other family?", a->packed16_floats, arithmetic,
                  (unsigned)decoder_packed16_floats(arithmetic));
    if (M == 0) return 0;
    MIPSF_REQUIRE((flags & ~(uint32_t)(MIPSF_WGRAD_LEAN_DACT | MIPSF_WGRAD_DETERMINISTIC)) == 0u, "unknown flags 0x%x", flags);
    const uint32_t lean_dact = (flags & MIPSF_WGRAD_LEAN_DACT) ? 1u : 0u;
    MIPSF_REQUIRE(!lean_dact || (packed16 != nullptr && (arithmetic == MIPSF_PREC_F16X3 || arithmetic == MIPSF_PREC_BF16X6)),
                  "the lean gradient record is read by the f16x3 / bf16x6 kernel with packed16 only");
    MIPSF_REQUIRE(packed16 == nullptr || arithmetic == MIPSF_PREC_F16X3 || arithmetic == MIPSF_PREC_BF16X6,
                  "H1 is recomputed by the f16x3 / bf16x6 arithmetic only (packed16 of the same family)");
    MIPSF_REQUIRE(feat && x && saved && dact && partial && grads, "null pointer");
    MIPSF_REQUIRE(feat_layout == MIPSF_FEAT_AOS || feat_layout == MIPSF_FEAT_LEVEL_MAJOR, "bad layout");
    MIPSF_REQUIRE(arithmetic == MIPSF_PREC_F16X3 || arithmetic == MIPSF_PREC_BF16X6 || arithmetic == MIPSF_PREC_BF16X3,
                  "arithmetic must be f16x3, bf16x6 or bf16x3");
    MIPSF_REQUIRE(M < (1u << 25), "M = %u: the grid features are addressed through one 4 GB buffer resource", M);
    hipStream_t s = (hipStream_t)stream;
    const bool det = (flags & MIPSF_WGRAD_DETERMINISTIC) != 0u;
    const uint64_t saved_bytes = (((uint64_t)M + 127) / 128) * 4 * ACT_TILE_FLOATS * 4;
    if (live_list != nullptr) {
        MIPSF_REQUIRE(packed16 != nullptr && (arithmetic == MIPSF_PREC_F16X3 || arithmetic == MIPSF_PREC_BF16X6),
                      "a live-sample list is read by the transpose-read exchange form only (f16x3 / bf16x6 with packed16)");
        MIPSF_REQUIRE(saved_bytes < (1ull << 32), "a live-sample list: the forward's record of %llu bytes is addressed through one "
                      "buffer resource of less than 4 GiB", (unsigned long long)saved_bytes);
        tile_live = nullptr;
    }
    if (det && tile_live)
        if (int e = decoder_tile_lists_order(const_cast<uint32_t*>(tile_live), M, s)) return e;
    const uint32_t n_tiles = (uint32_t)(((uint64_t)M + 31) / 32);
    const uint64_t n_bt = ((uint64_t)M + 127) / 128;
    const float* dsmall = dact + n_bt * 4 * ACT_TILE_FLOATS;
    const int cus = device_cus();
    if (cus <= 0) return 3;
    uint32_t blocks = n_tiles < (uint32_t)cus ? n_tiles : (uint32_t)cus;
    if (blocks > (uint32_t)W16_MAX_BLOCKS) blocks = (uint32_t)W16_MAX_BLOCKS;
    const uint32_t* live = tile_live;
    const int rc = with_layout(feat_layout, [&](auto LAY) {
        auto arm = [&](auto AR, auto RECOMP, auto CP) {
            hipLaunchKernelGGL((decoder_wgrad16_kernel<LAY.value, decltype(AR), RECOMP.value, CP.value>), dim3(blocks), dim3(W16_BLOCK), 0,
                               s, packed16, feat, x, saved, dact, dsmall, partial, M, n_tiles, live, lean_dact, live_list,
                               (uint32_t)saved_bytes);
            return check_launch("decoder_wgrad16");
        };
        constexpr ArF16 f16;
        constexpr ArBF3 bf3;
        constexpr ArBF2 bf2;
        if (live_list) return arithmetic == MIPSF_PREC_F16X3 ? arm(f16, yes, yes) : arm(bf3, yes, yes);
        if (arithmetic == MIPSF_PREC_F16X3) return packed16 ? arm(f16, yes, no) : arm(f16, no, no);
        if (arithmetic == MIPSF_PREC_BF16X6) return packed16 ? arm(bf3, yes, no) : arm(bf3, no, no);
        return arm(bf2, no, no);
    });
    if (rc) return rc;
    return wgrad_reduce_launch(partial, blocks, grads, s, det);
}
```

### mipsfusion_amd/model/scene_rep.py

```python
import copy

import numpy as np
import os
import torch
import torch.nn as nn

from .. import ops
from .._lib import FEAT_LEVEL_MAJOR
from .decoder import MLP_reg
from .encodings import get_encoder


class _PlaceFn(torch.autograd.Function):

    @staticmethod
    def forward(ctx, rays_o, rays_d, target_d, noise, tables, rc, N, S):
        rays_o, rays_d = ops._f32c(rays_o), ops._f32c(rays_d)
        z_vals, xn, counts = ops.sample_rays(rays_o, rays_d, target_d, noise, tables, rc, N, S)
        ctx.rc, ctx.N, ctx.S = rc, N, S
        ctx.save_for_backward(z_vals)
        ctx.mark_non_differentiable(z_vals, counts)
        ctx.set_materialize_grads(False)
        return z_vals, xn, counts

# ... 10 lines not shown

    @staticmethod
    def forward(ctx, pts, rc):
        ctx.rc = rc
        return ops.normalise_points(ops._f32c(pts), rc)

    @staticmethod
    def backward(ctx, dxn):
        return ops.normalise_bwd(ops._f32c(dxn), ctx.rc), None


_ROUTE_AHEAD_MIN_M = 65536
_MAX_QUERY, _QUERY_CHUNK = 1 << 24, 1 << 23


class _QueryFn(torch.autograd.Function):

    @staticmethod
    def forward(ctx, xn, owner, grid_params, ray_mask, *weights):
        xn = ops._f32c(xn)
        M = xn.shape[0]
        meta = owner.embed_fn.meta
        jac = None
        routed = None
        if ctx.needs_input_grad[2] and owner.route_ahead and M >= _ROUTE_AHEAD_MIN_M and not ops.resolve_deterministic(owner.deterministic):
            routed = ops.hashgrid_route_ahead(xn, meta)
        if ctx.needs_input_grad[0]:
            feat, jac = ops.hashgrid_fwd(xn, grid_params.detach(), meta, FEAT_LEVEL_MAJOR, with_jac=True, ray_mask=ray_mask)
        else:
            feat = ops.hashgrid_fwd(xn, grid_params.detach(), meta, FEAT_LEVEL_MAJOR)
        need = any(ctx.needs_input_grad)
        prec = owner.decoder_precision
        if prec == "f16" and need:
            raise RuntimeError('decoder_precision "f16" is forward-only (use "bf16x6", "f16x3" or "f32" when gradients are needed)')
        cache = owner._frozen_pack
        if cache is not None and prec in cache:
            packed, packed16 = cache[prec]
        else:
            if prec == "f32":
                packed, packed16 = ops.decoder_pack(weights), None
            else:
                packed, packed16 = None, ops.decoder_pack16(weights, precision=prec)
            if cache is not None:
                cache[prec] = (packed, packed16)
        lean = bool(need and prec in ops.SPLIT_PRECISIONS and owner.wgrad_precision in ("auto", "stream_" + prec) and owner.lean_record)
        masks_only = bool(need and prec in ops.SPLIT_PRECISIONS and not any(ctx.needs_input_grad[4:]))
        out, saved = ops.decoder_fwd(packed, feat, FEAT_LEVEL_MAJOR, xn, None, M,
                                     save="masks" if masks_only else ("lean" if lean else need), precision=prec, packed16=packed16)
        ctx.lean = lean and not masks_only
        ctx.tile_live = getattr(saved, "mipsf_tile_live", None)
        if packed is None:
            packed = packed16
        ctx.prec = prec
        if routed is not None:
            torch.cuda.current_stream(xn.device).wait_event(routed[1])
        ctx.routed = routed
        ctx.owner, ctx.M, ctx.meta, ctx.has_jac = owner, M, meta, jac is not None
        ctx.ray_mask = ray_mask if jac is not None else None
        ctx.save_for_backward(xn, feat, out, saved, packed, grid_params, *weights, *([jac] if jac is not None else []))
        return out

    @staticmethod
    def backward(ctx, dout):
        xn, feat, out, saved, packed, grid_params, *weights = ctx.saved_tensors
        jac = weights.pop() if ctx.has_jac else None
        need_w = any(ctx.needs_input_grad[4:])
        need_g = ctx.needs_input_grad[2]
        need_x = ctx.needs_input_grad[0]
        if ctx.tile_live is not None:
            saved.mipsf_tile_live = ctx.tile_live
        det = ops.resolve_deterministic(ctx.owner.deterministic)
        direct = ctx.owner.accumulate_param_grads_in_place and all(
            p.is_leaf and not p._backward_hooks for p in (grid_params, *weights))
        grads = None
        if need_w:
            grads = []
            for w, need in zip(weights, ctx.needs_input_grad[4:]):
                if direct and need:
                    if w.grad is None:
                        w.grad = torch.zeros_like(w)
                    grads.append(w.grad)
                else:
                    grads.append(torch.zeros_like(w))
        dfeat, dx, _, tiles = ops.decoder_bwd(packed, feat, FEAT_LEVEL_MAJOR, xn, None, out, ops._f32c(dout), saved, grads,
                                              ctx.M, precision=ctx.prec, packed16=packed if ctx.prec != "f32" else None,
                                              wgrad_precision=("stream_" + ctx.prec) if ctx.lean else ctx.owner.wgrad_precision,
                                              recompute_h1=ctx.lean, return_tiles=True, deterministic=det)
        dparams = None
        fresh_grad = False
        if need_g:
            if direct:
                if grid_params.grad is None:
                    grid_params.grad = torch.zeros_like(grid_params)
                    fresh_grad = True
                dparams = grid_params.grad
            else:
                dparams = torch.zeros_like(grid_params)
        if need_g:
            ops.hashgrid_bwd(xn, grid_params.detach(), dfeat, dparams, ctx.meta, FEAT_LEVEL_MAJOR, None, routed=ctx.routed,
                             dparams_zero=(not direct) or fresh_grad or ctx.owner.grid_grad_is_zero_at_backward, deterministic=det)
            ctx.routed = None
        if need_x:
            ops.hashgrid_dx_from_jac(jac, dfeat, dx, ctx.meta, FEAT_LEVEL_MAJOR, tiles=tiles,
                                     ray_mask=ctx.ray_mask)
        w_out = [None] * len(weights)
        if need_w and not direct:
            w_out = [g if need else None for g, need in zip(grads, ctx.needs_input_grad[4:])]
        return (dx if need_x else None, None, None if direct else dparams, None, *w_out)


class _RenderFn(torch.autograd.Function):
    fuse_backward = os.environ.get("MIPSF_RENDER_FUSE_BWD", "1") != "0"

    @staticmethod
    def forward(ctx, raw, z_vals, target_rgb, target_d, counts, rc, N, S, train, loss_w=None, share_of=None):
        raw = ops._f32c(raw)
        total = None
        ctx.n_norm = None
        ctx.draw, ctx.draw_stale = None, False
        if train and share_of is not None:
            rgb, depth, var, disp, acc, _, losses, total, ctx.n_norm = ops.render_fwd(
                raw, z_vals, target_rgb, target_d, counts, rc, N, S, train, loss_weights=loss_w, share_of=share_of)
        elif train and loss_w is not None:
            if ctx.needs_input_grad[0] and S <= ops.RENDER_DRAW_MAX_S and _RenderFn.fuse_backward:
                rgb, depth, var, disp, acc, _, losses, total, ctx.draw = ops.render_fwd(
                    raw, z_vals, target_rgb, target_d, counts, rc, N, S, train, loss_weights=loss_w, want_draw=True)
            else:
                rgb, depth, var, disp, acc, _, losses, total = ops.render_fwd(raw, z_vals, target_rgb, target_d, counts, rc, N,
                                                                              S, train, loss_weights=loss_w)
        else:
            rgb, depth, var, disp, acc, _, losses = ops.render_fwd(raw, z_vals, target_rgb, target_d, counts, rc, N, S,
                                                                   train)
        ctx.rc, ctx.N, ctx.S, ctx.train = rc, N, S, train
        ctx.save_for_backward(raw, z_vals, target_rgb, target_d, counts, losses, loss_w if total is not None else None)
        ctx.mark_non_differentiable(var, disp, acc)
        ctx.set_materialize_grads(False)
        if total is not None:
            return rgb, depth, var, disp, acc, losses, total.reshape(())
        if train:
            return rgb, depth, var, disp, acc, losses
        return rgb, depth, var, disp, acc

    @staticmethod
    def backward(ctx, g_rgb, g_depth, _gv, _gd, _ga, g_losses=None, g_total=None):
        raw, z_vals, target_rgb, target_d, counts, losses, loss_w = ctx.saved_tensors
        g_rgb = ops._f32c(g_rgb) if g_rgb is not None else None
        g_depth = ops._f32c(g_depth) if g_depth is not None else None
        g_total = ops._f32c(g_total).reshape(1) if (g_total is not None and loss_w is not None) else None
        if ctx.draw is not None and not ctx.draw_stale and g_total is not None and g_losses is None and g_rgb is None and g_depth is None:
            one = ops.unit_grad(raw.device)
            if g_total.data_ptr() == one.data_ptr() and one._version == 0:
                return ctx.draw, None, None, None, None, None, None, None, None, None, None
            ctx.draw_stale = True
            draw = ops.render_bwd(raw, z_vals, target_rgb, target_d, counts, losses, ctx.rc, None, None, None, ctx.N, ctx.S,
                                  g_total=g_total, loss_weights=loss_w, keep_draw=ctx.draw)
            return draw, None, None, None, None, None, None, None, None, None, None
        if ctx.train and g_losses is None and g_total is None:
            g_losses = torch.zeros(8, dtype=torch.float32, device=raw.device)
        draw = ops.render_bwd(raw, z_vals, target_rgb, target_d, counts, losses, ctx.rc,
                              ops._f32c(g_losses) if (ctx.train and g_losses is not None) else None, g_rgb, g_depth,
                              ctx.N, ctx.S, g_total=g_total, loss_weights=loss_w, n_norm=ctx.n_norm)
        return draw, None, None, None, None, None, None, None, None, None, None


class JointEncoding(nn.Module):
    def __init__(self, config, bound_box, coords_norm_factor):
        super().__init__()
        self.config = config
        self.bounding_box = bound_box
        self.coords_norm_factor = coords_norm_factor
        self._bound64 = torch.as_tensor(bound_box).detach().to("cpu", torch.float64).tolist()
        self._half64 = torch.as_tensor(coords_norm_factor).detach().to("cpu", torch.float64).reshape(-1).tolist()
        self.accumulate_param_grads_in_place = False
        self.grid_grad_is_zero_at_backward = False
        self.deterministic = None
        self.decoder_precision = "bf16x6"
        self.wgrad_precision = "auto"
        self.lean_record = True
        self.route_ahead = False
        self.mask_fixed_rays = os.environ.get("MIPSF_NO_DX_MASK", "0") != "1"
        self.ray_share_reduce = None
        self._frozen_pack = None
        self._tables = {}
        self._jitter_ring = {}
        self.get_resolution()
        self.get_encoding(config)
        self.get_decoder(config)
        self.save_initial_param()

    def get_resolution(self):
        dim_max = max(b[1] - b[0] for b in self._bound64)
# ... 213 lines not shown
```

### mipsfusion_amd/ops.py

```python
from __future__ import annotations

import ctypes as C
import os
from typing import Optional

import torch

from . import _lib
from ._lib import FEAT_AOS, FEAT_LEVEL_MAJOR, check, dptr, lib, stream_ptr

DECODER_PARAM_ORDER = ("pts_linear.0.weight", "pts_linear.0.bias", "pts_linear.2.weight", "pts_linear.2.bias",
                       "rgb_linear.0.weight", "rgb_linear.0.bias", "sdf_linear.0.weight", "sdf_linear.0.bias",
                       "sdf_linear.2.weight", "sdf_linear.2.bias")
_DEC_FIELDS = ("w_pts0", "b_pts0", "w_pts2", "b_pts2", "w_rgb0", "b_rgb0", "w_sdf0", "b_sdf0", "w_sdf2", "b_sdf2")
_DEC_SHAPES = ((128, 51), (128,), (128, 128), (128,), (3, 115), (3,), (128, 96), (128,), (5, 128), (5,))


PROFILE = None


class _timed:
    def __init__(self, name, stream=None):
        self.name, self.stream = name, stream

# ... 108 lines not shown
    if key not in _SIDE_STREAMS:
        _SIDE_STREAMS[key] = torch.cuda.Stream(device=key)
    return _SIDE_STREAMS[key]


def hashgrid_route_ahead(x, meta):
    M = x.shape[0]
    n = _lib.buffer_size(_lib.SIZE_HASHGRID_BWD_SCRATCH, M, 0, 0, meta)
    scratch = torch.empty(n, dtype=torch.float32, device=x.device)
    main, side = torch.cuda.current_stream(x.device), side_stream(x.device)
    side.wait_stream(main)
    with _timed("hashgrid_route", side):
        check(lib().mipsf_hashgrid_route(dptr(x), dptr(scratch), M, C.byref(meta), C.c_void_p(side.cuda_stream)),
              "hashgrid_route")
    ev = torch.cuda.Event()
    ev.record(side)
    return scratch, ev


_ZEROED = {}
_lib.KEPT_BLOCK_CACHES.append(_ZEROED)


def _zeroed_words(device, n, tag):
    key = (device.index, stream_ptr(), tag, n)
    buf = _ZEROED.get(key)
    if buf is None:
        buf = _ZEROED[key] = torch.zeros(n, dtype=torch.int32, device=device)
    return buf


_SCATTER_COUNTERS = {}
_lib.KEPT_BLOCK_CACHES.append(_SCATTER_COUNTERS)


def _scatter_counters(device, meta):
    n = _lib.buffer_size(_lib.SIZE_HASHGRID_COUNTER_WORDS, meta=meta)
    key = (device.index, stream_ptr(), n)
    buf = _SCATTER_COUNTERS.get(key)
    if buf is None:
        buf = _SCATTER_COUNTERS[key] = torch.zeros(n, dtype=torch.int32, device=device)
    return buf


LEAN_DACT = not bool(os.environ.get("MIPSF_FULL_DACT"))
HG_DPARAMS_ZERO = 1
HG_ROUTED = 2
HG_DETERMINISTIC = 4
_HG_IGNORE_ZERO_HINT = bool(os.environ.get("MIPSF_HG_IGNORE_ZERO_HINT"))


def hashgrid_bwd(x, params, dout, dparams, meta, layout=FEAT_AOS, dx: Optional[torch.Tensor] = None, routed=None,
                 dparams_zero=False, deterministic=False):
    M = x.shape[0]
    if PROFILE is not None:
        global _LAST_SCATTER_DOUT
        _LAST_SCATTER_DOUT = dout
    a = _lib.HashgridBwdArgs.new(M=M, x=dptr(x), params=dptr(params), dout=dptr(dout), dparams=dptr(dparams),
                                 meta=C.pointer(meta), feat_layout=layout)
    if deterministic:
        if routed is not None:
            torch.cuda.current_stream(x.device).wait_event(routed[1])
        n = _lib.buffer_size(_lib.SIZE_HASHGRID_DET_SCRATCH, M, 1 if dx is not None else 0, 0, meta)
        scratch = torch.empty(n, dtype=torch.float32, device=x.device)
        a.dx, a.scratch = dptr(dx), dptr(scratch)
        a.flags = HG_DETERMINISTIC | (HG_DPARAMS_ZERO if (dparams_zero and not _HG_IGNORE_ZERO_HINT) else 0)
        with _timed("hashgrid_bwd"):
            check(lib().mipsf_hashgrid_bwd(C.byref(a), stream_ptr()), "hashgrid_bwd (deterministic)")
        return
    if routed is not None and dx is None and dparams is not None:
        scratch, ev = routed
        torch.cuda.current_stream(x.device).wait_event(ev)
        a.scratch, a.flags = dptr(scratch), HG_ROUTED
        with _timed("hashgrid_bwd"):
            check(lib().mipsf_hashgrid_bwd(C.byref(a), stream_ptr()), "hashgrid_bwd (routed)")
        return
    n = _lib.buffer_size(_lib.SIZE_HASHGRID_BWD_SCRATCH, M, 1 if dx is not None else 0, 0, meta)
    scratch = torch.empty(n, dtype=torch.float32, device=x.device)
    counters = _scatter_counters(x.device, meta)
    a.dx, a.scratch, a.counters = dptr(dx), dptr(scratch), dptr(counters, torch.int32)
    a.flags = HG_DPARAMS_ZERO if (dparams_zero and not _HG_IGNORE_ZERO_HINT) else 0
    with _timed("hashgrid_bwd"):
        check(lib().mipsf_hashgrid_bwd(C.byref(a), stream_ptr()), "hashgrid_bwd")


def hashgrid_indices(x, meta) -> torch.Tensor:
    M = x.shape[0]
    idx = torch.empty((M, meta.n_levels, 8), dtype=torch.int32, device=x.device)
    check(lib().mipsf_hashgrid_indices(dptr(x), dptr(idx, torch.int32), M, C.byref(meta), stream_ptr()),
          "hashgrid_indices")
    return idx


def resolve_deterministic(flag) -> bool:
    return torch.are_deterministic_algorithms_enabled() if flag is None else bool(flag)


class HashGridFn(torch.autograd.Function):

    @staticmethod
    def forward(ctx, x, params, meta, deterministic=None):
        x = _f32c(x)
        ctx.meta = meta
        ctx.deterministic = deterministic
        if ctx.needs_input_grad[0]:
            out, jac = hashgrid_fwd(x, params.detach(), meta, FEAT_AOS, with_jac=True)
            ctx.save_for_backward(x, params, jac)
            return out
        ctx.save_for_backward(x, params)
        return hashgrid_fwd(x, params.detach(), meta, FEAT_AOS)

    @staticmethod
    def backward(ctx, dout):
        x, params, *jac = ctx.saved_tensors
        dout = _f32c(dout)
        dparams = torch.zeros_like(params) if ctx.needs_input_grad[1] else None
        dx = torch.zeros_like(x) if ctx.needs_input_grad[0] else None
        if dparams is not None:
            hashgrid_bwd(x, params.detach(), dout, dparams, ctx.meta, FEAT_AOS, None, dparams_zero=True,
                         deterministic=resolve_deterministic(ctx.deterministic))
        if dx is not None:
            hashgrid_dx_from_jac(jac[0], dout, dx, ctx.meta, FEAT_AOS)
        return dx, dparams, None, None


class FrequencyFn(torch.autograd.Function):
    @staticmethod
    def forward(ctx, x, n_freq):
        x = _f32c(x)
        ctx.n_freq = n_freq
        ctx.save_for_backward(x)
        M, D = x.shape
        out = torch.empty((M, D * 2 * n_freq), dtype=torch.float32, device=x.device)
        check(lib().mipsf_freq_fwd(dptr(x), dptr(out), M, D, n_freq, stream_ptr()), "freq_fwd")
        return out

    @staticmethod
    def backward(ctx, dout):
        (x,) = ctx.saved_tensors
        M, D = x.shape
        dx = torch.empty_like(x)
        check(lib().mipsf_freq_bwd(dptr(x), dptr(_f32c(dout)), dptr(dx), M, D, ctx.n_freq, stream_ptr()),
              "freq_bwd")
        return dx, None


def _decoder_struct(tensors, cls):
    st = cls()
    for field, t, shape in zip(_DEC_FIELDS, tensors, _DEC_SHAPES):
        if tuple(t.shape) != shape:
            raise RuntimeError(f"decoder tensor {field} has shape {tuple(t.shape)}, expected {shape}")
        setattr(st, field, dptr(t))
    return st


def decoder_pack(weights, packed: Optional[torch.Tensor] = None) -> torch.Tensor:
    dev = weights[0].device
    if packed is None:
        packed = torch.empty(_lib.buffer_size(_lib.SIZE_DECODER_PACKED), dtype=torch.float32, device=dev)
    ws = [w.detach() for w in weights]
    st = _decoder_struct(ws, _lib.DecoderWeights)
    with _timed("decoder_pack"):
        check(lib().mipsf_decoder_pack(C.byref(st), dptr(packed), stream_ptr()), "decoder_pack")
    return packed


def decoder_pack16(weights, packed16: Optional[torch.Tensor] = None, precision: str = "f16x3") -> torch.Tensor:
    dev = weights[0].device
    fam = _PACK16_FAMILY[precision]
    n = _lib.buffer_size(_lib.SIZE_DECODER_PACKED16, 0, _lib.PREC[fam])
    if packed16 is None:
        packed16 = torch.empty(n, dtype=torch.float32, device=dev)
    elif packed16.numel() != n:
        raise RuntimeError(f"packed16 has {packed16.numel()} floats, precision {precision!r} needs {n}")
    st = _decoder_struct([w.detach() for w in weights], _lib.DecoderWeights)
    with _timed("decoder_pack"):
        check(lib().mipsf_decoder_pack16(C.byref(st), dptr(packed16), _lib.PREC[fam], stream_ptr()), "decoder_pack16")
    packed16.mipsf_family = fam
    return packed16


_PACK16_FAMILY = {"f16x3": "f16x3", "f16": "f16x3", "bf16x6": "bf16x6"}
SPLIT_PRECISIONS = ("f16x3", "bf16x6")


def _check_family(packed16, precision):
    fam = getattr(packed16, "mipsf_family", None)
    if fam is not None and fam != _PACK16_FAMILY[precision]:
        raise RuntimeError(f"packed16 was packed for {fam!r}, the call asks for {precision!r}")
    n = _lib.buffer_size(_lib.SIZE_DECODER_PACKED16, 0, _lib.PREC[_PACK16_FAMILY[precision]])
    if packed16.numel() != n:
        raise RuntimeError(f"packed16 holds {packed16.numel()} floats, precision {precision!r} needs {n}: packed for the other family?")


def decoder_fwd(packed, feat, layout, x, embed_pos, M, save, precision: str = "f32", packed16=None):
    lean = save in ("lean", "masks")
    masks_only = save == "masks"
    if lean and precision not in SPLIT_PRECISIONS:
        raise RuntimeError('save="lean" / "masks" belong to precision "f16x3" / "bf16x6"')
    out = torch.empty((M, 10), dtype=torch.float32, device=x.device)
    saved = None
    if save:
        saved = torch.empty(_lib.buffer_size(_lib.SIZE_DECODER_SAVED, M), dtype=torch.float32, device=x.device)
    if precision != "f32":
        if embed_pos is not None or packed16 is None:
            raise RuntimeError("the f16 decoder modes take packed16 and compute the positional encoding in-kernel")
        if save and precision not in SPLIT_PRECISIONS:
            raise RuntimeError('only precision "f32" / "f16x3" / "bf16x6" keep activations for the backward pass')
        _check_family(packed16, precision)
        tile_live = None
        if save and SKIP_ZERO_TILES:
            tile_live = torch.empty(_lib.buffer_size(_lib.SIZE_DECODER_TILE_WORDS, M), dtype=torch.int32, device=x.device)
        a = _lib.DecoderFwd16Args.new(M=M, packed16=dptr(packed16), feat=dptr(feat), x=dptr(x), out=dptr(out), saved=dptr(saved),
                                      tile_live_clear=dptr(tile_live, torch.int32), feat_layout=layout,
                                      precision=_lib.PREC[precision], lean_record=(2 if masks_only else 1) if lean else 0,
                                      packed16_floats=packed16.numel())
        with _timed("decoder_fwd"):
            check(lib().mipsf_decoder_fwd16(C.byref(a), stream_ptr()), "decoder_fwd16")
        if lean:
            saved.mipsf_lean_record = True
        if masks_only:
            saved.mipsf_masks_only = True
        if tile_live is not None:
            saved.mipsf_tile_live = [tile_live, True]
        return out, saved
    pe_mode = 0 if embed_pos is None else 1
    with _timed("decoder_fwd"):
        check(lib().mipsf_decoder_fwd(dptr(packed), dptr(feat), layout, dptr(x), dptr(embed_pos), pe_mode, dptr(out),
                                      dptr(saved), M, stream_ptr()), "decoder_fwd")
    return out, saved


def decoder_bwd(packed, feat, layout, x, embed_pos, out, dout, saved, grads, M, precision: str = "f32", packed16=None,
                wgrad_precision: str = "auto", recompute_h1: bool = False, return_tiles: bool = False,
                deterministic: bool = False):
    if wgrad_precision == "auto":
        wgrad_precision = ("stream_" + precision) if (precision in SPLIT_PRECISIONS and embed_pos is None) else "f32"
    if getattr(saved, "mipsf_masks_only", False) and grads is not None:
        raise RuntimeError("this activation record holds the ReLU masks only (decoder_fwd(save='masks')): no weight gradients")
    if getattr(saved, "mipsf_lean_record", False) and grads is not None:
        if wgrad_precision not in ("stream_f16x3", "stream_bf16x6") or packed16 is None or wgrad_precision != "stream_" + precision:
            raise RuntimeError("this activation record was saved lean (no H1): the weight gradients need the streaming kernel "
                               "of the forward's arithmetic (wgrad_precision='stream_f16x3' / 'stream_bf16x6') with packed16 "
                               "(H1 is recomputed from x)")
        recompute_h1 = True
    dev = x.device
    dfeat = torch.empty_like(feat)
    dx = torch.empty((M, 3), dtype=torch.float32, device=dev)
    dpe = torch.empty((M, 48), dtype=torch.float32, device=dev) if embed_pos is not None else None
    dact = None if (grads is None and precision in SPLIT_PRECISIONS) else torch.empty(_lib.buffer_size(_lib.SIZE_DECODER_DACT, M), dtype=torch.float32, device=dev)
    pe_mode = 0 if embed_pos is None else 1
    tile_live = None
    live_list = None
    lean_dact = False
    if precision in SPLIT_PRECISIONS:
        if embed_pos is not None or packed16 is None:
            raise RuntimeError("the f16x3 / bf16x6 backward chain takes packed16 and computes the positional encoding in-kernel")
        _check_family(packed16, precision)
        hdr_clear = 4 if precision == "bf16x6" else 0
        lean_dact = bool(LEAN_DACT and grads is not None and wgrad_precision == "stream_" + precision and recompute_h1
                         and packed16 is not None)
        if SKIP_ZERO_TILES and (grads is None or wgrad_precision.startswith("stream_")):
            global _LAST_TILE_LIVE
            pre = getattr(saved, "mipsf_tile_live", None)
            if pre is not None and pre[1]:
                tile_live, hdr_clear = pre[0], hdr_clear | 1
                pre[1] = False
            else:
                tile_live = torch.empty(_lib.buffer_size(_lib.SIZE_DECODER_TILE_WORDS, M), dtype=torch.int32, device=dev)
            _LAST_TILE_LIVE = (tile_live, M, False)
            exchange = wgrad_precision == "stream_" + precision and recompute_h1 and packed16 is not None
            if (COMPACT_LIVE and (grads is None or exchange)
                    and _lib.buffer_size(_lib.SIZE_DECODER_SAVED, M) * 4 < (1 << 32)):
                live_list = torch.empty(_lib.buffer_size(_lib.SIZE_DECODER_LIVE_LIST, M), dtype=torch.int32, device=dev)
                _LAST_TILE_LIVE = (live_list, M, True)
                with _timed("decoder_bwd_chain"):
                    check(lib().mipsf_decoder_live_compact(dptr(dout), M, dptr(live_list, torch.int32), dptr(dfeat), dptr(dx),
                                                           layout, stream_ptr()), "decoder_live_compact")
        a = _lib.DecoderChain16Args.new(live_list=dptr(live_list, torch.int32), M=M, packed16=dptr(packed16), x=dptr(x), out=dptr(out), dout=dptr(dout), saved=dptr(saved),
                                        dfeat=dptr(dfeat), dx=dptr(dx), dact=dptr(dact), tile_live=dptr(tile_live, torch.int32),
                                        feat_layout=layout, flags=hdr_clear | (2 if lean_dact else 0), packed16_floats=packed16.numel())
        with _timed("decoder_bwd_chain"):
            check(lib().mipsf_decoder_bwd_chain16(C.byref(a), stream_ptr()), "decoder_bwd_chain16")
    else:
        with _timed("decoder_bwd_chain"):
            check(lib().mipsf_decoder_bwd_chain(dptr(packed), layout, dptr(x), pe_mode, dptr(out), dptr(dout),
                                                dptr(saved), dptr(dfeat), dptr(dx), dptr(dpe), dptr(dact), M,
                                                stream_ptr()), "decoder_bwd_chain")
    tiles = LiveList(live_list) if live_list is not None else tile_live
    if grads is not None:
        partial = torch.empty(_lib.buffer_size(_lib.SIZE_DECODER_WGRAD_PARTIAL), dtype=torch.float32, device=dev)
        st = _decoder_struct(grads, _lib.DecoderGrads)
        if wgrad_precision.startswith("stream_"):
            if embed_pos is not None:
                raise RuntimeError("the streaming weight-gradient kernel computes the positional encoding in-kernel")
            arith = _lib.PREC[wgrad_precision[len("stream_"):]]
            if recompute_h1 and (wgrad_precision not in ("stream_f16x3", "stream_bf16x6") or packed16 is None):
                raise RuntimeError("recompute_h1 needs wgrad_precision 'stream_f16x3' / 'stream_bf16x6' and packed16")
            if recompute_h1:
                _check_family(packed16, wgrad_precision[len("stream_"):])
            a = _lib.DecoderWgrad16Args.new(live_list=dptr(live_list, torch.int32),
                                            M=M, packed16=dptr(packed16) if recompute_h1 else None, feat=dptr(feat), x=dptr(x),
                                            saved=dptr(saved), dact=dptr(dact), tile_live=dptr(tile_live, torch.int32),
                                            grads=C.pointer(st), partial=dptr(partial), feat_layout=layout, arithmetic=arith,
                                            flags=(_lib.WGRAD_LEAN_DACT if lean_dact else 0)
                                            | (_lib.WGRAD_DETERMINISTIC if deterministic else 0),
                                            packed16_floats=packed16.numel() if recompute_h1 else 0)
            with _timed("decoder_wgrad"):
                check(lib().mipsf_decoder_wgrad16(C.byref(a), stream_ptr()), "decoder_wgrad16")
            return (dfeat, dx, dpe, tiles) if return_tiles else (dfeat, dx, dpe)
        if recompute_h1:
            raise RuntimeError("recompute_h1 needs wgrad_precision 'stream_f16x3'")
        if deterministic:
            raise RuntimeError("deterministic training needs the streaming weight-gradient kernel (decoder_precision 'bf16x6' / "
                               "'f16x3', wgrad_precision 'auto' or 'stream_*'): the fp32 kernel's reduce adds in float atomics")
        with _timed("decoder_wgrad"):
            wprec = _lib.PREC[wgrad_precision]
            check(lib().mipsf_decoder_wgrad(dptr(feat), layout, dptr(x), dptr(embed_pos), pe_mode, dptr(saved),
                                            dptr(dact), C.byref(st), dptr(partial), wprec, M, stream_ptr()),
                  "decoder_wgrad")
    return (dfeat, dx, dpe, tiles) if return_tiles else (dfeat, dx, dpe)


def decoder_fwd_sdf(packed, feat, layout, x, embed_pos, M, precision: str = "f32", packed16=None) -> torch.Tensor:
    sdf = torch.empty((M,), dtype=torch.float32, device=x.device)
    if precision != "f32":
        if embed_pos is not None or packed16 is None:
            raise RuntimeError("the f16 decoder modes take packed16 and compute the positional encoding in-kernel")
        _check_family(packed16, precision)
        with _timed("decoder_fwd"):
            a = _lib.DecoderFwd16Args.new(M=M, packed16=dptr(packed16), feat=dptr(feat), x=dptr(x), out=dptr(sdf), feat_layout=layout,
                                          precision=_lib.PREC[precision], sdf_only=1, packed16_floats=packed16.numel())
            check(lib().mipsf_decoder_fwd16(C.byref(a), stream_ptr()), "decoder_fwd16")
        return sdf
    pe_mode = 0 if embed_pos is None else 1
    with _timed("decoder_fwd"):
        check(lib().mipsf_decoder_fwd_sdf(dptr(packed), dptr(feat), layout, dptr(x), dptr(embed_pos), pe_mode, dptr(sdf),
                                          M, stream_ptr()), "decoder_fwd_sdf")
    return sdf


class DecoderFn(torch.autograd.Function):

    @staticmethod
    def forward(ctx, embed, embed_pos, x, *weights):
        embed, embed_pos, x = _f32c(embed), _f32c(embed_pos), _f32c(x)
        M = x.shape[0]
        packed = decoder_pack(weights)
        need = any(ctx.needs_input_grad)
        out, saved = decoder_fwd(packed, embed, FEAT_AOS, x, embed_pos, M, save=need)
        ctx.M = M
        ctx.save_for_backward(embed, embed_pos, x, out, saved, packed, *weights)
        return out

    @staticmethod
    def backward(ctx, dout):
        embed, embed_pos, x, out, saved, packed, *weights = ctx.saved_tensors
        need_w = any(ctx.needs_input_grad[3:])
        grads = [torch.zeros_like(w) for w in weights] if need_w else None
        dfeat, dx, dpe = decoder_bwd(packed, embed, FEAT_AOS, x, embed_pos, out, _f32c(dout), saved, grads, ctx.M)
        return (dfeat, dpe, dx, *(grads if need_w else [None] * len(weights)))


def make_render_cfg(cfg: dict, bound64, half_len64, n_uniform: int, n_near: int, emd_w: float) -> _lib.RenderCfg:
    tr, cam = cfg["training"], cfg["cam"]
    rc = _lib.RenderCfg()
    rc.n_uniform, rc.n_near = n_uniform, n_near
    rc.perturb = 1 if tr["perturb"] > 0.0 else 0
    rc.use_bound = 1 if cfg["grid"]["use_bound_normalize"] else 0
    for d in range(3):
        rc.bound_min[d] = float(bound64[d][0])
        rc.bound_max[d] = float(bound64[d][1])
        rc.half_len[d] = float(half_len64[d])
    if not cfg["grid"]["tcnn_encoding"]:
        raise RuntimeError("grid.tcnn_encoding = False is not a configuration the reference ships")
    rc.norm_factor = float(tr["norm_factor"])
    rc.trunc = float(tr["trunc"])
    rc.sc_factor = float(cfg["data"]["sc_factor"])
    rc.depth_trunc = float(cam["depth_trunc"])
    rc.rgb_missing_nonzero = 1 if tr["rgb_missing"] != 0 else 0
    rc.emd_w = float(emd_w)
    return rc


def normalise_points(pts: torch.Tensor, rc) -> torch.Tensor:
    xn = torch.empty_like(pts)
    check(lib().mipsf_normalise_points(dptr(pts), C.byref(rc), dptr(xn), pts.shape[0], stream_ptr()), "normalise")
    return xn


def normalise_bwd(dxn: torch.Tensor, rc) -> torch.Tensor:
    dpts = torch.empty_like(dxn)
# ... 375 lines not shown
```

Before: 456.0 million rays*samples/s.

## Fuse hashgrid scatter, dx-from-jacobian and decoder weight-grad reduce into one backward tail kernel

Adds a single backward_tail kernel that runs the hash-grid scatter route, the dx-from-jacobian pass and the decoder weight-gradient reduce as virtual blocks inside one launch. The decoder wgrad16 kernel now skips its own reduce and hands the partial records on to this tail. It also rewrites the weight-grad reduce to accumulate per-slice sums in double and combine them in shared memory. The aim is to remove launch overhead and serialisation between small tail kernels, at the cost of mixing heterogeneous work in one grid and taking on more code complexity.

```diff
diff --git a/include/mipsf_compact.h b/include/mipsf_compact.h
--- a/include/mipsf_compact.h
+++ b/include/mipsf_compact.h
@@ -27,6 +27,32 @@
                                       const uint32_t* live_list, const uint32_t* ray_mask, uint32_t S, uint32_t M,
                                       const mipsf_grid_meta* meta_host, int layout, void* stream);
 
+typedef struct mipsf_backward_tail_args {
+    uint32_t struct_size;
+    uint32_t M;
+    const float* x;
+    const float* dout;
+    float* dparams;
+    float* scratch;
+    uint32_t* counters;
+    const mipsf_grid_meta* meta;
+    int feat_layout;
+    uint32_t flags;
+    const float* jac;
+    float* dx;
+    const uint32_t* tile_live;
+    const uint32_t* live_list;
+    const uint32_t* ray_mask;
+    uint32_t S;
+    uint32_t n_records;
+    const float* partial;
+    const mipsf_decoder_grads* grads;
+} mipsf_backward_tail_args;
+int mipsf_backward_tail(const mipsf_backward_tail_args* args_host, void* stream);
+
+#define MIPSF_WGRAD_NO_REDUCE 4u
+uint32_t mipsf_decoder_wgrad16_records(uint32_t M);
+
 #ifdef __cplusplus
 }
 #endif
diff --git a/mipsfusion_amd/_lib.py b/mipsfusion_amd/_lib.py
--- a/mipsfusion_amd/_lib.py
+++ b/mipsfusion_amd/_lib.py
@@ -171,7 +171,14 @@
                                   ("capacity_tris", _CU)])
 McubesWeldArgs = _args("McubesWeldArgs", [("T", _CU), ("soup", _VP), ("scratch", _VP), ("vertices", _VP), ("faces", _VP),
                                           ("counts", _VP), ("max_rounds", _CU)])
+WGRAD_NO_REDUCE = 4
+BackwardTailArgs = _args("BackwardTailArgs", [("M", _CU), ("x", _VP), ("dout", _VP), ("dparams", _VP), ("scratch", _VP), ("counters", _VP),
+                                              ("meta", C.POINTER(GridMeta)), ("feat_layout", _CI), ("flags", _CU), ("jac", _VP),
+                                              ("dx", _VP), ("tile_live", _VP), ("live_list", _VP), ("ray_mask", _VP), ("S", _CU),
+                                              ("n_records", _CU), ("partial", _VP), ("grads", C.POINTER(DecoderGrads))])
 COMPACT_SIGNATURES = {
+    "mipsf_backward_tail": (_I, [C.POINTER(BackwardTailArgs), _P]),
+    "mipsf_decoder_wgrad16_records": (_U32, [_U32]),
     "mipsf_decoder_live_compact": (_I, [_P, _U32, _P, _P, _P, _I, _P]),
     "mipsf_hashgrid_dx_from_jac_list": (_I, [_P, _P, _P, _P, _U32, C.POINTER(GridMeta), _I, _P]),
     "mipsf_gather_pose_place_fwd_masked": (_I, [_P, _U64, _P, _P, _P, _P, _U32, _U32, _P, _P, _P, _P, _P, C.POINTER(RenderCfg),
diff --git a/mipsfusion_amd/csrc/decoder.hip b/mipsfusion_amd/csrc/decoder.hip
--- a/mipsfusion_amd/csrc/decoder.hip
+++ b/mipsfusion_amd/csrc/decoder.hip
@@ -1,4 +1,5 @@
 #include "decoder_dev.h"
+#include "wgrad_reduce_dev.h"
 #include "launch.h"
 
 namespace mipsf {
@@ -782,30 +783,10 @@
 }
 
 
-struct GradPtrs {
-    float* p[10];
-};
-
-constexpr int WG_REDUCE_SLICES = 8;
-__global__ __launch_bounds__(256) void decoder_wgrad_reduce_kernel(const float* __restrict__ partial, uint32_t nrec,
-                                                                   GradPtrs g) {
-    const int q = blockIdx.x * blockDim.x + threadIdx.x;
-    if (q >= G_TOTAL) return;
-    float a0 = 0.f, a1 = 0.f, a2 = 0.f, a3 = 0.f;
-    uint32_t b = blockIdx.y;
-    for (; b + 3 * WG_REDUCE_SLICES < nrec; b += 4 * WG_REDUCE_SLICES) {
-        a0 += partial[(size_t)b * G_STRIDE + q];
-        a1 += partial[(size_t)(b + WG_REDUCE_SLICES) * G_STRIDE + q];
-        a2 += partial[(size_t)(b + 2 * WG_REDUCE_SLICES) * G_STRIDE + q];
-        a3 += partial[(size_t)(b + 3 * WG_REDUCE_SLICES) * G_STRIDE + q];
-    }
-    for (; b < nrec; b += WG_REDUCE_SLICES) a0 += partial[(size_t)b * G_STRIDE + q];
-    const float a = (a0 + a1) + (a2 + a3);
-    const int bounds[11] = {G_W_PTS0, G_B_PTS0, G_W_PTS2, G_B_PTS2, G_W_RGB0, G_B_RGB0,
-                            G_W_SDF0, G_B_SDF0, G_W_SDF2, G_B_SDF2, G_TOTAL};
-#pragma unroll
-    for (int k = 0; k < 10; ++k)
-        if (q >= bounds[k] && q < bounds[k + 1]) unsafeAtomicAdd(&g.p[k][q - bounds[k]], a);
+__global__ __launch_bounds__(WG_REDUCE_BLOCK) void decoder_wgrad_reduce_kernel(const float* __restrict__ partial, uint32_t nrec,
+                                                                               GradPtrs g) {
+    __shared__ double sh[WG_REDUCE_BLOCK];
+    wgrad_reduce_block(blockIdx.x, threadIdx.x, true, partial, nrec, g, sh);
 }
 
 __global__ __launch_bounds__(256) void decoder_pack_kernel(W w, float* __restrict__ packed) {
@@ -822,30 +803,16 @@
 
 constexpr uint32_t WG_MAX_BLOCKS = 256;
 
-__global__ __launch_bounds__(256) void decoder_wgrad_reduce_fixed_kernel(const float* __restrict__ partial, uint32_t nrec,
-                                                                         GradPtrs g) {
-    const int q = blockIdx.x * blockDim.x + threadIdx.x;
-    if (q >= G_TOTAL) return;
-    float a = 0.f;
-    for (uint32_t b = 0; b < nrec; ++b) a += partial[(size_t)b * G_STRIDE + q];
-    const int bounds[11] = {G_W_PTS0, G_B_PTS0, G_W_PTS2, G_B_PTS2, G_W_RGB0, G_B_RGB0,
-                            G_W_SDF0, G_B_SDF0, G_W_SDF2, G_B_SDF2, G_TOTAL};
-#pragma unroll
-    for (int k = 0; k < 10; ++k)
-        if (q >= bounds[k] && q < bounds[k + 1]) {
-            float* p = &g.p[k][q - bounds[k]];
-            *p = *p + a;
-        }
+__global__ __launch_bounds__(WG_REDUCE_BLOCK) void decoder_wgrad_reduce_fixed_kernel(const float* __restrict__ partial, uint32_t nrec,
+                                                                                     GradPtrs g) {
+    wgrad_reduce_fixed_block(blockIdx.x, threadIdx.x, partial, nrec, g);
 }
 
 int wgrad_reduce_launch(const float* partial, uint32_t nrec, const mipsf_decoder_grads* grads, hipStream_t s, bool fixed_order) {
     if (fixed_order) {
         GradPtrs g;
-        g.p[0] = grads->w_pts0, g.p[1] = grads->b_pts0, g.p[2] = grads->w_pts2, g.p[3] = grads->b_pts2;
-        g.p[4] = grads->w_rgb0, g.p[5] = grads->b_rgb0, g.p[6] = grads->w_sdf0, g.p[7] = grads->b_sdf0;
-        g.p[8] = grads->w_sdf2, g.p[9] = grads->b_sdf2;
-        for (int k = 0; k < 10; ++k) MIPSF_REQUIRE(g.p[k] != nullptr, "null gradient pointer %d", k);
-        hipLaunchKernelGGL(decoder_wgrad_reduce_fixed_kernel, dim3((G_TOTAL + 255) / 256), dim3(256), 0, s, partial, nrec, g);
+        MIPSF_REQUIRE(wgrad_grad_ptrs(grads, g), "null gradient pointer");
+        hipLaunchKernelGGL(decoder_wgrad_reduce_fixed_kernel, dim3(WG_REDUCE_BLOCKS_X), dim3(WG_REDUCE_BLOCK), 0, s, partial, nrec, g);
         return check_launch("decoder_wgrad_reduce_fixed");
     }
     return wgrad_reduce_launch(partial, nrec, grads, s);
@@ -853,12 +820,9 @@
 
 int wgrad_reduce_launch(const float* partial, uint32_t nrec, const mipsf_decoder_grads* grads, hipStream_t s) {
     GradPtrs g;
-    g.p[0] = grads->w_pts0, g.p[1] = grads->b_pts0, g.p[2] = grads->w_pts2, g.p[3] = grads->b_pts2;
-    g.p[4] = grads->w_rgb0, g.p[5] = grads->b_rgb0, g.p[6] = grads->w_sdf0, g.p[7] = grads->b_sdf0;
-    g.p[8] = grads->w_sdf2, g.p[9] = grads->b_sdf2;
-    for (int k = 0; k < 10; ++k) MIPSF_REQUIRE(g.p[k] != nullptr, "null gradient pointer %d", k);
-    hipLaunchKernelGGL(decoder_wgrad_reduce_kernel, dim3((G_TOTAL + 255) / 256, WG_REDUCE_SLICES), dim3(256), 0, s, partial,
-                       nrec, g);
+    MIPSF_REQUIRE(wgrad_grad_ptrs(grads, g), "null gradient pointer");
+    hipLaunchKernelGGL(decoder_wgrad_reduce_kernel, dim3(WG_REDUCE_VBLOCKS), dim3(WG_REDUCE_BLOCK), 0, s,
+                       partial, nrec, g);
     return check_launch("decoder_wgrad_reduce");
 }
 
@@ -968,10 +932,7 @@
     const uint32_t n_bt = (uint32_t)n_block_tiles(M);
     const float* dsmall = dact + n_block_tiles(M) * 4 * ACT_TILE_FLOATS;
     GradPtrs g;
-    g.p[0] = grads->w_pts0, g.p[1] = grads->b_pts0, g.p[2] = grads->w_pts2, g.p[3] = grads->b_pts2;
-    g.p[4] = grads->w_rgb0, g.p[5] = grads->b_rgb0, g.p[6] = grads->w_sdf0, g.p[7] = grads->b_sdf0;
-    g.p[8] = grads->w_sdf2, g.p[9] = grads->b_sdf2;
-    for (int k = 0; k < 10; ++k) MIPSF_REQUIRE(g.p[k] != nullptr, "null gradient pointer %d", k);
+    MIPSF_REQUIRE(wgrad_grad_ptrs(grads, g), "null gradient pointer");
     const int cus = device_cus();
     if (cus <= 0) return 3;
     uint32_t wg_blocks = n_bt < (uint32_t)cus ? n_bt : (uint32_t)cus;
@@ -986,7 +947,7 @@
         });
     }); });
     if (rc) return rc;
-    hipLaunchKernelGGL(decoder_wgrad_reduce_kernel, dim3((G_TOTAL + 255) / 256, WG_REDUCE_SLICES), dim3(256), 0, s, partial, wg_blocks, g);
+    hipLaunchKernelGGL(decoder_wgrad_reduce_kernel, dim3(WG_REDUCE_VBLOCKS), dim3(WG_REDUCE_BLOCK), 0, s, partial, wg_blocks, g);
     return check_launch("decoder_wgrad_reduce");
 }
 
diff --git a/mipsfusion_amd/csrc/hashgrid.hip b/mipsfusion_amd/csrc/hashgrid.hip
--- a/mipsfusion_amd/csrc/hashgrid.hip
+++ b/mipsfusion_amd/csrc/hashgrid.hip
@@ -1,6 +1,7 @@
 #include "common.h"
 #include "launch.h"
 #include "decoder_layout.h"
+#include "wgrad_reduce_dev.h"
 
 namespace mipsf {
 
@@ -349,10 +350,10 @@
 __host__ __device__ inline uint32_t route_groups(uint32_t n_levels) { return (n_levels + RT_LEVELS - 1) / RT_LEVELS; }
 
 template <int LAYOUT>
-__global__ __launch_bounds__(RT_BLOCK) void scatter_route_kernel(const float* __restrict__ x,
-                                                                const float* __restrict__ dout, uint32_t M, GridLevels g,
-                                                                ScatterPlan plan, uint32_t* __restrict__ ws,
-                                                                uint32_t* __restrict__ cw) {
+__device__ __forceinline__ void scatter_route_block(const uint32_t vblock, const float* __restrict__ x,
+                                                    const float* __restrict__ dout, uint32_t M, const GridLevels& g,
+                                                    const ScatterPlan& plan, uint32_t* __restrict__ ws,
+                                                    uint32_t* __restrict__ cw) {
     __shared__ uint32_t cnt[SC_MAX_NS];
     __shared__ uint32_t base[SC_MAX_NS];
 #ifndef MIPSF_SC_STAGE
@@ -365,8 +366,8 @@
     __shared__ uint32_t lstart[SC_MAX_NS];
     __shared__ uint32_t stage[MIPSF_SC_STAGE ? STAGE_CAP : 1];
     const uint32_t n_groups = route_groups(plan.n_levels);
-    const uint32_t group = blockIdx.x % n_groups;
-    const uint32_t chunk = blockIdx.x / n_groups;
+    const uint32_t group = vblock % n_groups;
+    const uint32_t chunk = vblock / n_groups;
 #ifndef MIPSF_SC_AGG_MAX
 #define MIPSF_SC_AGG_MAX 1
 #endif
@@ -582,11 +583,19 @@
     }
 #ifdef MIPSF_RT_TRACE
     if ((threadIdx.x & 63u) == 0u) {
-        unsigned long long* tr = reinterpret_cast<unsigned long long*>(ws + plan.w_end + 64) + (size_t)(blockIdx.x * (RT_BLOCK / 64) + (threadIdx.x >> 6)) * 10;
+        unsigned long long* tr = reinterpret_cast<unsigned long long*>(ws + plan.w_end + 64) + (size_t)(vblock * (RT_BLOCK / 64) + (threadIdx.x >> 6)) * 10;
         for (int q = 0; q < 9; ++q) tr[q] = tr_acc[q];
         tr[9] = (unsigned long long)(group | (tr_levels << 8));
     }
 #endif
+}
+
+template <int LAYOUT>
+__global__ __launch_bounds__(RT_BLOCK) void scatter_route_kernel(const float* __restrict__ x,
+                                                                const float* __restrict__ dout, uint32_t M, GridLevels g,
+                                                                ScatterPlan plan, uint32_t* __restrict__ ws,
+                                                                uint32_t* __restrict__ cw) {
+    scatter_route_block<LAYOUT>(blockIdx.x, x, dout, M, g, plan, ws, cw);
 }
 __device__ __forceinline__ uint32_t part_of(const ScatterPlan& plan, uint32_t bin) {
     return bin < plan.dense_bins ? SC_PART_DENSE : SC_PART;
@@ -1068,46 +1077,92 @@
     dx[t] += a;
 }
 
+constexpr uint32_t DX_BLOCK = 256;
 template <int LAYOUT>
-MIPSF_SINGLE_FP32 __global__ __launch_bounds__(256) void hashgrid_dx_jac_kernel(const float* __restrict__ jac,
+__device__ __forceinline__ void hashgrid_dx_jac_block(const uint32_t vblock, const uint32_t vthread, const float* __restrict__ jac,
+                                                      const float* __restrict__ dout, float* __restrict__ dx,
+                                                      uint32_t M, uint32_t L,
+                                                      const uint32_t* __restrict__ tiles,
+                                                      const uint32_t* __restrict__ live_list,
+                                                      const uint32_t* __restrict__ ray_mask, uint32_t S) {
+    uint32_t i = vblock * DX_BLOCK + vthread;
+    if (live_list != nullptr) {
+        if (i >= M || i >= live_list[0]) return;
+        i = live_list[MIPSF_LIVE_HEADER + i];
+    }
+    if (tiles != nullptr) {
+        const uint32_t k = i >> 5, cap = mipsf::dl::tl_cap((M + 31u) / 32u);
+        uint32_t q = 0, first = 0, total = 0;
+#pragma unroll
+        for (uint32_t j = 0; j < 8; ++j) {
+            const uint32_t n = tiles[64 * j + 32];
+            if (k >= total && n != 0u) q = j, first = total;
+            total += n;
+        }
+        if (k >= total) return;
+        i = tiles[mipsf::dl::TL_HEADER + q * cap + (k - first)] * 32u + (i & 31u);
+    }
+    if (i >= M) return;
+    if (!ray_wants_dx(ray_mask, S, i)) {
+        dx[3 * (size_t)i] = 0.f, dx[3 * (size_t)i + 1] = 0.f, dx[3 * (size_t)i + 2] = 0.f;
+        return;
+    }
+    float a[3] = {0.f, 0.f, 0.f};
+    for (uint32_t l = 0; l < L; ++l) {
+        const float2* j2 = reinterpret_cast<const float2*>(jac) + (size_t)l * 3 * M + i;
+        const float2 gy = *reinterpret_cast<const float2*>(dout + feat_index<LAYOUT>(i, l, M, L));
+#pragma unroll
+        for (int d = 0; d < 3; ++d) {
+            const float2 j = j2[(size_t)d * M];
+            a[d] += j.x * gy.x + j.y * gy.y;
+        }
+    }
+    dx[3 * (size_t)i] += a[0], dx[3 * (size_t)i + 1] += a[1], dx[3 * (size_t)i + 2] += a[2];
+}
+
+template <int LAYOUT>
+MIPSF_SINGLE_FP32 __global__ __launch_bounds__(DX_BLOCK) void hashgrid_dx_jac_kernel(const float* __restrict__ jac,
                                                               const float* __restrict__ dout, float* __restrict__ dx,
                                                               uint32_t M, uint32_t L,
                                                               const uint32_t* __restrict__ tiles,
                                                               const uint32_t* __restrict__ live_list,
                                                               const uint32_t* __restrict__ ray_mask, uint32_t S) {
-    uint32_t i = blockIdx.x * blockDim.x + threadIdx.x;
-    if (live_list != nullptr) {
-        if (i >= M || i >= live_list[0]) return;
-        i = live_list[MIPSF_LIVE_HEADER + i];
-    }
-    if (tiles != nullptr) {
-        const uint32_t k = i >> 5, cap = mipsf::dl::tl_cap((M + 31u) / 32u);
-        uint32_t q = 0, first = 0, total = 0;
-#pragma unroll
-        for (uint32_t j = 0; j < 8; ++j) {
-            const uint32_t n = tiles[64 * j + 32];
-            if (k >= total && n != 0u) q = j, first = total;
-            total += n;
-        }
-        if (k >= total) return;
-        i = tiles[mipsf::dl::TL_HEADER + q * cap + (k - first)] * 32u + (i & 31u);
-    }
-    if (i >= M) return;
-    if (!ray_wants_dx(ray_mask, S, i)) {
-        dx[3 * (size_t)i] = 0.f, dx[3 * (size_t)i + 1] = 0.f, dx[3 * (size_t)i + 2] = 0.f;
+    hashgrid_dx_jac_block<LAYOUT>(blockIdx.x, threadIdx.x, jac, dout, dx, M, L, tiles, live_list, ray_mask, S);
+}
+
+struct TailArgs {
+    const float* x;
+    const float* dout;
+    const float* route_dout;
+    uint32_t* ws;
+    uint32_t* cw;
+    const float* jac;
+    float* dx;
+    const uint32_t* tiles;
+    const uint32_t* live_list;
+    const uint32_t* ray_mask;
+    const float* partial;
+    GradPtrs grads;
+    uint32_t M, S, nrec, n_dx, n_red;
+};
+static_assert(RT_BLOCK == 2 * DX_BLOCK && RT_BLOCK == 2 * WG_REDUCE_BLOCK, "a tail workgroup runs two 256-thread virtual blocks");
+
+template <int LAYOUT>
+MIPSF_SINGLE_FP32 __global__ __launch_bounds__(RT_BLOCK) void backward_tail_kernel(TailArgs a, GridLevels g, ScatterPlan plan) {
+    const uint32_t b = blockIdx.x;
+    const uint32_t half = threadIdx.x / DX_BLOCK, vthread = threadIdx.x % DX_BLOCK;
+    if (b < a.n_dx) {
+        hashgrid_dx_jac_block<LAYOUT>(2u * b + half, vthread, a.jac, a.dout, a.dx, a.M, g.n_levels, a.tiles, a.live_list, a.ray_mask,
+                                      a.S);
         return;
     }
-    float a[3] = {0.f, 0.f, 0.f};
-    for (uint32_t l = 0; l < L; ++l) {
-        const float2* j2 = reinterpret_cast<const float2*>(jac) + (size_t)l * 3 * M + i;
-        const float2 gy = *reinterpret_cast<const float2*>(dout + feat_index<LAYOUT>(i, l, M, L));
-#pragma unroll
-        for (int d = 0; d < 3; ++d) {
-            const float2 j = j2[(size_t)d * M];
-            a[d] += j.x * gy.x + j.y * gy.y;
-        }
-    }
-    dx[3 * (size_t)i] += a[0], dx[3 * (size_t)i + 1] += a[1], dx[3 * (size_t)i + 2] += a[2];
+    if (b < a.n_dx + a.n_red) {
+        __shared__ double red[2 * WG_REDUCE_BLOCK];
+        const uint32_t v = 2u * (b - a.n_dx) + half;
+        wgrad_reduce_block(v, vthread, v < (uint32_t)WG_REDUCE_VBLOCKS, a.partial, a.nrec, a.grads, red + half * WG_REDUCE_BLOCK);
+        return;
+    }
+    scatter_route_block<LAYOUT>(b - a.n_dx - a.n_red, a.x, a.route_dout, a.M, g, plan, a.ws, a.cw);
 }
 
 __global__ __launch_bounds__(HG_BLOCK) void hashgrid_indices_kernel(const float* __restrict__ x,
@@ -1573,17 +1628,50 @@
     return 0;
 }
 
+static void launch_clear(uint32_t* cw, const ScatterPlan& plan, hipStream_t s) {
+    const uint32_t nz = plan.w_first;
+    hipLaunchKernelGGL(scatter_zero_kernel, dim3((nz + 255) / 256), dim3(256), 0, s, cw, nz);
+}
+static inline uint32_t route_blocks(const GridLevels& g, uint32_t M) {
+    return route_groups(g.n_levels) * ((M + RT_BLOCK * SC_ROUTE_UNR - 1) / (RT_BLOCK * SC_ROUTE_UNR));
+}
 static int launch_route(const float* x, const float* dout, int layout, uint32_t* ws, uint32_t* cw, bool clear, uint32_t M,
                         const GridLevels& g, const ScatterPlan& plan, hipStream_t s) {
-    if (clear) {
-        const uint32_t nz = plan.w_first;
-        hipLaunchKernelGGL(scatter_zero_kernel, dim3((nz + 255) / 256), dim3(256), 0, s, cw, nz);
-    }
-    const uint32_t rb = route_groups(g.n_levels) * ((M + RT_BLOCK * SC_ROUTE_UNR - 1) / (RT_BLOCK * SC_ROUTE_UNR));
+    if (clear) launch_clear(cw, plan, s);
+    const uint32_t rb = route_blocks(g, M);
     return with_layout(layout, [&](auto LAY) {
         hipLaunchKernelGGL(scatter_route_kernel<LAY.value>, dim3(rb), dim3(RT_BLOCK), 0, s, x, dout, M, g, plan, ws, cw);
         return check_launch("hashgrid_route");
     });
+}
+
+static int launch_accumulate(const float* x, const float* dout, float* dparams, int layout, uint32_t* ws, uint32_t* cw, uint32_t M,
+                             const GridLevels& g, const ScatterPlan& plan, hipStream_t s) {
+    const uint32_t lds_bytes = plan.max_slice * 16 + plan.n_bins * 4;
+    const int cus = device_cus();
+    if (cus <= 0) return 3;
+    uint32_t per_cu = (160u * 1024u) / (lds_bytes + 256u);
+    per_cu = per_cu < 1u ? 1u : (per_cu > 2048u / SC_BLOCK ? 2048u / SC_BLOCK : per_cu);
+    const uint32_t want = (uint32_t)cus * per_cu;
+    const uint32_t blocks = plan.max_items < want ? plan.max_items : want;
+    const int rc = with_layout(layout, [&](auto LAY) {
+        constexpr auto kern = hashgrid_scatter_persist_kernel<LAY.value>;
+        if (!grant_lds<kern>(lds_bytes)) return lds_refused(lds_bytes);
+        hipLaunchKernelGGL(kern, dim3(blocks), dim3(SC_BLOCK), lds_bytes, s, x, dout, dparams, M, g, plan, ws, cw);
+        return check_launch("hashgrid_scatter");
+    });
+    if (rc) return rc;
+    if (plan.fold_launch) {
+        hipLaunchKernelGGL(hashgrid_scatter_reduce_kernel, dim3(plan.n_bins, (plan.max_slice + 255) / 256), dim3(256), 0, s,
+                           dparams, g, plan, ws, cw);
+        if (int e = check_launch("hashgrid_scatter_reduce")) return e;
+    }
+    return 0;
+}
+
+static uint32_t fold_launch_wanted() {
+    const char* e = getenv("MIPSF_SC_FOLD_LAUNCH");
+    return (e && e[0] && e[0] != '0') ? 1u : 0u;
 }
 
 int mipsf_hashgrid_route(const float* x, float* scratch, uint32_t M, const mipsf_grid_meta* meta, void* stream) {
@@ -1609,10 +1697,7 @@
     hipStream_t s = (hipStream_t)stream;
     ScatterPlan plan = make_plan(g, M);
     plan.fresh = fresh ? 1u : 0u;
-    {
-        const char* e = getenv("MIPSF_SC_FOLD_LAUNCH");
-        plan.fold_launch = (e && e[0] && e[0] != '0') ? 1u : 0u;
-    }
+    plan.fold_launch = fold_launch_wanted();
     if (int rc = check_plan(plan, g, M)) return rc;
     uint32_t* ws = reinterpret_cast<uint32_t*>(scratch);
     uint32_t* cw = counters ? counters : ws;
@@ -1620,25 +1705,7 @@
     if (dparams) {
         if (!routed)
             if (int e = launch_route(x, MIPSF_SC_SKIP_ZERO ? dout : nullptr, layout, ws, cw, counters == nullptr, M, g, plan, s)) return e;
-        const uint32_t lds_bytes = plan.max_slice * 16 + plan.n_bins * 4;
-        const int cus = device_cus();
-        if (cus <= 0) return 3;
-        uint32_t per_cu = (160u * 1024u) / (lds_bytes + 256u);
-        per_cu = per_cu < 1u ? 1u : (per_cu > 2048u / SC_BLOCK ? 2048u / SC_BLOCK : per_cu);
-        const uint32_t want = (uint32_t)cus * per_cu;
-        const uint32_t blocks = plan.max_items < want ? plan.max_items : want;
-        const int rc = with_layout(layout, [&](auto LAY) {
-            constexpr auto kern = hashgrid_scatter_persist_kernel<LAY.value>;
-            if (!grant_lds<kern>(lds_bytes)) return lds_refused(lds_bytes);
-            hipLaunchKernelGGL(kern, dim3(blocks), dim3(SC_BLOCK), lds_bytes, s, x, dout, dparams, M, g, plan, ws, cw);
-            return check_launch("hashgrid_scatter");
-        });
-        if (rc) return rc;
-        if (plan.fold_launch) {
-            hipLaunchKernelGGL(hashgrid_scatter_reduce_kernel, dim3(plan.n_bins, (plan.max_slice + 255) / 256), dim3(256), 0, s,
-                               dparams, g, plan, ws, cw);
-            if (int e = check_launch("hashgrid_scatter_reduce")) return e;
-        }
+        if (int e = launch_accumulate(x, dout, dparams, layout, ws, cw, M, g, plan, s)) return e;
     }
     if (dx) return launch_dx(x, params, dout, dxl, dx, M, g, layout, s);
     return 0;
@@ -1660,6 +1727,51 @@
                              (a->flags & MIPSF_HG_ROUTED) != 0u, stream, (a->flags & MIPSF_HG_DPARAMS_ZERO) != 0u);
 }
 
+int mipsf_backward_tail(const mipsf_backward_tail_args* a, void* stream) {
+    MIPSF_REQUIRE(a != nullptr, "null argument block");
+    MIPSF_REQUIRE(a->struct_size == sizeof(mipsf_backward_tail_args), "mipsf_backward_tail_args: struct_size %u, this library expects %u",
+                  a->struct_size, (unsigned)sizeof(mipsf_backward_tail_args));
+    MIPSF_REQUIRE((a->flags & ~(uint32_t)MIPSF_HG_DPARAMS_ZERO) == 0u, "unknown flags 0x%x", a->flags);
+    GridLevels g;
+    if (int rc = to_levels(a->meta, g)) return rc;
+    const uint32_t M = a->M;
+    if (M == 0) return 0;
+    MIPSF_REQUIRE(a->x && a->dout && a->dparams && a->scratch, "null pointer");
+    const int layout = a->feat_layout;
+    MIPSF_REQUIRE(layout == MIPSF_FEAT_AOS || layout == MIPSF_FEAT_LEVEL_MAJOR, "bad layout %d", layout);
+    TailArgs t = {};
+    if (a->jac != nullptr) {
+        MIPSF_REQUIRE(a->dx != nullptr, "null dx");
+        MIPSF_REQUIRE(!(a->tile_live && a->live_list), "tile_live and live_list are alternatives");
+        if (int rc = check_ray_mask(a->ray_mask, a->S, M)) return rc;
+        t.jac = a->jac, t.dx = a->dx, t.tiles = a->tile_live, t.live_list = a->live_list, t.ray_mask = a->ray_mask, t.S = a->S;
+        t.n_dx = (M + RT_BLOCK - 1) / RT_BLOCK;
+    }
+    if (a->partial != nullptr) {
+        MIPSF_REQUIRE(a->grads != nullptr && wgrad_grad_ptrs(a->grads, t.grads), "null gradient pointer");
+        MIPSF_REQUIRE(a->n_records >= 1u && (uint64_t)a->n_records * dl::G_STRIDE <= decoder_wgrad_partial_floats(),
+                      "n_records = %u: not what a weight-gradient call leaves", a->n_records);
+        t.partial = a->partial, t.nrec = a->n_records;
+        t.n_red = (uint32_t)(WG_REDUCE_VBLOCKS + 1) / 2u;
+    }
+    hipStream_t s = (hipStream_t)stream;
+    ScatterPlan plan = make_plan(g, M);
+    plan.fresh = (a->flags & MIPSF_HG_DPARAMS_ZERO) ? 1u : 0u;
+    plan.fold_launch = fold_launch_wanted();
+    if (int rc = check_plan(plan, g, M)) return rc;
+    uint32_t* ws = reinterpret_cast<uint32_t*>(a->scratch);
+    uint32_t* cw = a->counters ? a->counters : ws;
+    if (a->counters == nullptr) launch_clear(cw, plan, s);
+    t.x = a->x, t.dout = a->dout, t.route_dout = MIPSF_SC_SKIP_ZERO ? a->dout : nullptr, t.ws = ws, t.cw = cw, t.M = M;
+    const uint32_t blocks = t.n_dx + t.n_red + route_blocks(g, M);
+    const int rc = with_layout(layout, [&](auto LAY) {
+        hipLaunchKernelGGL(backward_tail_kernel<LAY.value>, dim3(blocks), dim3(RT_BLOCK), 0, s, t, g, plan);
+        return check_launch("backward_tail");
+    });
+    if (rc) return rc;
+    return launch_accumulate(a->x, a->dout, a->dparams, layout, ws, cw, M, g, plan, s);
+}
+
 int mipsf_hashgrid_indices(const float* x, uint32_t* idx, uint32_t M, const mipsf_grid_meta* meta, void* stream) {
     GridLevels g;
     if (int rc = to_levels(meta, g)) return rc;
diff --git a/mipsfusion_amd/csrc/wgrad16.hip b/mipsfusion_amd/csrc/wgrad16.hip
--- a/mipsfusion_amd/csrc/wgrad16.hip
+++ b/mipsfusion_amd/csrc/wgrad16.hip
@@ -1286,6 +1286,11 @@
 uint64_t decoder_tile_words(uint32_t M) { return TL_HEADER + 8ull * tl_cap((uint32_t)(((uint64_t)M + 31) / 32)); }
 }
 
+static uint32_t w16_blocks(uint32_t n_tiles, int cus) {
+    const uint32_t blocks = n_tiles < (uint32_t)cus ? n_tiles : (uint32_t)cus;
+    return blocks > (uint32_t)W16_MAX_BLOCKS ? (uint32_t)W16_MAX_BLOCKS : blocks;
+}
+
 extern "C" int mipsf_decoder_wgrad16(const mipsf_decoder_wgrad16_args* a, void* stream) {
     MIPSF_REQUIRE(a != nullptr, "null argument block");
     MIPSF_REQUIRE(a->struct_size == sizeof(mipsf_decoder_wgrad16_args), "mipsf_decoder_wgrad16_args: struct_size %u, this library expects %u",
@@ -1299,7 +1304,10 @@
                   "packed16 holds %u floats, arithmetic %d needs %u: packed for the other family?", a->packed16_floats, arithmetic,
                   (unsigned)decoder_packed16_floats(arithmetic));
     if (M == 0) return 0;
-    MIPSF_REQUIRE((flags & ~(uint32_t)(MIPSF_WGRAD_LEAN_DACT | MIPSF_WGRAD_DETERMINISTIC)) == 0u, "unknown flags 0x%x", flags);
+    MIPSF_REQUIRE((flags & ~(uint32_t)(MIPSF_WGRAD_LEAN_DACT | MIPSF_WGRAD_DETERMINISTIC | MIPSF_WGRAD_NO_REDUCE)) == 0u,
+                  "unknown flags 0x%x", flags);
+    MIPSF_REQUIRE((flags & (MIPSF_WGRAD_DETERMINISTIC | MIPSF_WGRAD_NO_REDUCE)) != (MIPSF_WGRAD_DETERMINISTIC | MIPSF_WGRAD_NO_REDUCE),
+                  "MIPSF_WGRAD_NO_REDUCE leaves the records to mipsf_backward_tail, whose reduce is not the ordered one");
     const uint32_t lean_dact = (flags & MIPSF_WGRAD_LEAN_DACT) ? 1u : 0u;
     MIPSF_REQUIRE(!lean_dact || (packed16 != nullptr && (arithmetic == MIPSF_PREC_F16X3 || arithmetic == MIPSF_PREC_BF16X6)),
                   "the lean gradient record is read by the f16x3 / bf16x6 kernel with packed16 only");
@@ -1327,8 +1335,7 @@
     const float* dsmall = dact + n_bt * 4 * ACT_TILE_FLOATS;
     const int cus = device_cus();
     if (cus <= 0) return 3;
-    uint32_t blocks = n_tiles < (uint32_t)cus ? n_tiles : (uint32_t)cus;
-    if (blocks > (uint32_t)W16_MAX_BLOCKS) blocks = (uint32_t)W16_MAX_BLOCKS;
+    const uint32_t blocks = w16_blocks(n_tiles, cus);
     const uint32_t* live = tile_live;
     const int rc = with_layout(feat_layout, [&](auto LAY) {
         auto arm = [&](auto AR, auto RECOMP, auto CP) {
@@ -1346,5 +1353,13 @@
         return arm(bf2, no, no);
     });
     if (rc) return rc;
+    if (flags & MIPSF_WGRAD_NO_REDUCE) return 0;
     return wgrad_reduce_launch(partial, blocks, grads, s, det);
 }
+
+extern "C" uint32_t mipsf_decoder_wgrad16_records(uint32_t M) {
+    if (M == 0) return 0;
+    const int cus = device_cus();
+    if (cus <= 0) return 0;
+    return w16_blocks((uint32_t)(((uint64_t)M + 31) / 32), cus);
+}
diff --git a/mipsfusion_amd/csrc/wgrad_reduce_dev.h b/mipsfusion_amd/csrc/wgrad_reduce_dev.h
--- /dev/null
+++ b/mipsfusion_amd/csrc/wgrad_reduce_dev.h
@@ -0,0 +1,73 @@
+#pragma once
+#include "common.h"
+#include "decoder_layout.h"
+
+namespace mipsf {
+
+struct GradPtrs {
+    float* p[10];
+};
+
+constexpr int WG_REDUCE_SLICES = 8;
+constexpr int WG_REDUCE_BLOCK = 256;
+constexpr int WG_REDUCE_BLOCKS_X = (dl::G_TOTAL + WG_REDUCE_BLOCK - 1) / WG_REDUCE_BLOCK;
+constexpr int WG_REDUCE_ELEMS = WG_REDUCE_BLOCK / WG_REDUCE_SLICES;
+constexpr int WG_REDUCE_VBLOCKS = (dl::G_TOTAL + WG_REDUCE_ELEMS - 1) / WG_REDUCE_ELEMS;
+
+template <class Add>
+__device__ __forceinline__ void wgrad_reduce_store(const GradPtrs& g, int q, float a, Add add) {
+    using namespace dl;
+    const int bounds[11] = {G_W_PTS0, G_B_PTS0, G_W_PTS2, G_B_PTS2, G_W_RGB0, G_B_RGB0,
+                            G_W_SDF0, G_B_SDF0, G_W_SDF2, G_B_SDF2, G_TOTAL};
+#pragma unroll
+    for (int k = 0; k < 10; ++k)
+        if (q >= bounds[k] && q < bounds[k + 1]) add(&g.p[k][q - bounds[k]], a);
+}
+
+__device__ __forceinline__ void wgrad_reduce_block(uint32_t vblock, uint32_t vthread, bool active, const float* __restrict__ partial,
+                                                   uint32_t nrec, const GradPtrs& g, double* sh) {
+    using namespace dl;
+    const uint32_t e = vthread % WG_REDUCE_ELEMS, slice = vthread / WG_REDUCE_ELEMS;
+    const int q = (int)(vblock * WG_REDUCE_ELEMS + e);
+    const bool mine = active && q < G_TOTAL;
+    double a0 = 0.0, a1 = 0.0, a2 = 0.0, a3 = 0.0;
+    if (mine) {
+        uint32_t b = slice;
+        for (; b + 3 * WG_REDUCE_SLICES < nrec; b += 4 * WG_REDUCE_SLICES) {
+            a0 += (double)partial[(size_t)b * G_STRIDE + q];
+            a1 += (double)partial[(size_t)(b + WG_REDUCE_SLICES) * G_STRIDE + q];
+            a2 += (double)partial[(size_t)(b + 2 * WG_REDUCE_SLICES) * G_STRIDE + q];
+            a3 += (double)partial[(size_t)(b + 3 * WG_REDUCE_SLICES) * G_STRIDE + q];
+        }
+        for (; b < nrec; b += WG_REDUCE_SLICES) a0 += (double)partial[(size_t)b * G_STRIDE + q];
+    }
+    sh[vthread] = (a0 + a1) + (a2 + a3);
+    __syncthreads();
+    if (mine && slice == 0u) {
+        double t = 0.0;
+#pragma unroll
+        for (int s = 0; s < WG_REDUCE_SLICES; ++s) t += sh[s * WG_REDUCE_ELEMS + e];
+        wgrad_reduce_store(g, q, (float)t, [](float* p, float v) { unsafeAtomicAdd(p, v); });
+    }
+}
+
+__device__ __forceinline__ void wgrad_reduce_fixed_block(uint32_t vbx, uint32_t vthread, const float* __restrict__ partial,
+                                                         uint32_t nrec, const GradPtrs& g) {
+    using namespace dl;
+    const int q = vbx * WG_REDUCE_BLOCK + vthread;
+    if (q >= G_TOTAL) return;
+    float a = 0.f;
+    for (uint32_t b = 0; b < nrec; ++b) a += partial[(size_t)b * G_STRIDE + q];
+    wgrad_reduce_store(g, q, a, [](float* p, float v) { *p = *p + v; });
+}
+
+inline bool wgrad_grad_ptrs(const mipsf_decoder_grads* grads, GradPtrs& g) {
+    g.p[0] = grads->w_pts0, g.p[1] = grads->b_pts0, g.p[2] = grads->w_pts2, g.p[3] = grads->b_pts2;
+    g.p[4] = grads->w_rgb0, g.p[5] = grads->b_rgb0, g.p[6] = grads->w_sdf0, g.p[7] = grads->b_sdf0;
+    g.p[8] = grads->w_sdf2, g.p[9] = grads->b_sdf2;
+    for (int k = 0; k < 10; ++k)
+        if (g.p[k] == nullptr) return false;
+    return true;
+}
+
+}
diff --git a/mipsfusion_amd/model/scene_rep.py b/mipsfusion_amd/model/scene_rep.py
--- a/mipsfusion_amd/model/scene_rep.py
+++ b/mipsfusion_amd/model/scene_rep.py
@@ -116,10 +116,14 @@
                     grads.append(w.grad)
                 else:
                     grads.append(torch.zeros_like(w))
+        roles = ops.tail_roles() if (need_g and need_x and need_w and ctx.lean and not det and ctx.routed is None) else 0
+        deferred = {} if roles & 2 else None
         dfeat, dx, _, tiles = ops.decoder_bwd(packed, feat, FEAT_LEVEL_MAJOR, xn, None, out, ops._f32c(dout), saved, grads,
                                               ctx.M, precision=ctx.prec, packed16=packed if ctx.prec != "f32" else None,
                                               wgrad_precision=("stream_" + ctx.prec) if ctx.lean else ctx.owner.wgrad_precision,
-                                              recompute_h1=ctx.lean, return_tiles=True, deterministic=det)
+                                              recompute_h1=ctx.lean, return_tiles=True, deterministic=det, defer_reduce=deferred)
+        if not isinstance(tiles, ops.LiveList):
+            roles = 0
         dparams = None
         fresh_grad = False
         if need_g:
@@ -130,9 +134,14 @@
                 dparams = grid_params.grad
             else:
                 dparams = torch.zeros_like(grid_params)
+        zero = (not direct) or fresh_grad or ctx.owner.grid_grad_is_zero_at_backward
+        if roles:
+            ops.backward_tail(xn, dfeat, dparams, ctx.meta, FEAT_LEVEL_MAJOR,
+                              dx_args=(jac, dx, tiles, ctx.ray_mask) if roles & 1 else None, deferred=deferred, dparams_zero=zero)
+            need_g, need_x = False, need_x and not roles & 1
         if need_g:
             ops.hashgrid_bwd(xn, grid_params.detach(), dfeat, dparams, ctx.meta, FEAT_LEVEL_MAJOR, None, routed=ctx.routed,
-                             dparams_zero=(not direct) or fresh_grad or ctx.owner.grid_grad_is_zero_at_backward, deterministic=det)
+                             dparams_zero=zero, deterministic=det)
             ctx.routed = None
         if need_x:
             ops.hashgrid_dx_from_jac(jac, dfeat, dx, ctx.meta, FEAT_LEVEL_MAJOR, tiles=tiles,
@@ -140,7 +149,7 @@
         w_out = [None] * len(weights)
         if need_w and not direct:
             w_out = [g if need else None for g, need in zip(grads, ctx.needs_input_grad[4:])]
-        return (dx if need_x else None, None, None if direct else dparams, None, *w_out)
+        return (dx if ctx.needs_input_grad[0] else None, None, None if direct else dparams, None, *w_out)
 
 
 class _RenderFn(torch.autograd.Function):
diff --git a/mipsfusion_amd/ops.py b/mipsfusion_amd/ops.py
--- a/mipsfusion_amd/ops.py
+++ b/mipsfusion_amd/ops.py
@@ -214,6 +214,38 @@
     a.flags = HG_DPARAMS_ZERO if (dparams_zero and not _HG_IGNORE_ZERO_HINT) else 0
     with _timed("hashgrid_bwd"):
         check(lib().mipsf_hashgrid_bwd(C.byref(a), stream_ptr()), "hashgrid_bwd")
+
+
+def tail_roles() -> int:
+    if os.environ.get("MIPSF_NO_TAIL_FUSE", "0") not in ("", "0"):
+        return 0
+    return int(os.environ.get("MIPSF_TAIL_ROLES", "3")) & 3
+
+
+def backward_tail(x, dfeat, dparams, meta, layout, dx_args=None, deferred=None, dparams_zero=False):
+    M = x.shape[0]
+    if PROFILE is not None:
+        global _LAST_SCATTER_DOUT
+        _LAST_SCATTER_DOUT = dfeat
+    n = _lib.buffer_size(_lib.SIZE_HASHGRID_BWD_SCRATCH, M, 0, 0, meta)
+    scratch = torch.empty(n, dtype=torch.float32, device=x.device)
+    counters = _scatter_counters(x.device, meta)
+    a = _lib.BackwardTailArgs.new(M=M, x=dptr(x), dout=dptr(dfeat), dparams=dptr(dparams), scratch=dptr(scratch),
+                                  counters=dptr(counters, torch.int32), meta=C.pointer(meta), feat_layout=layout,
+                                  flags=HG_DPARAMS_ZERO if (dparams_zero and not _HG_IGNORE_ZERO_HINT) else 0)
+    if dx_args is not None:
+        jac, dx, tiles, ray_mask = dx_args
+        if ray_mask is not None and (ray_mask.shape[0] == 0 or M % ray_mask.shape[0] != 0):
+            raise RuntimeError(f"ray mask: {M} samples are not whole rays of {ray_mask.shape[0]} rays")
+        lst = isinstance(tiles, LiveList)
+        a.jac, a.dx = dptr(jac), dptr(dx)
+        a.tile_live = None if lst else dptr(tiles, torch.int32)
+        a.live_list = dptr(tiles.buf, torch.int32) if lst else None
+        a.ray_mask, a.S = dptr(ray_mask, torch.int32), (M // ray_mask.shape[0] if ray_mask is not None else 0)
+    if deferred:
+        a.partial, a.n_records, a.grads = dptr(deferred["partial"]), deferred["n_records"], C.pointer(deferred["grads"])
+    with _timed("hashgrid_bwd"):
+        check(lib().mipsf_backward_tail(C.byref(a), stream_ptr()), "backward_tail")
 
 
 def hashgrid_indices(x, meta) -> torch.Tensor:
@@ -365,7 +397,7 @@
 
 def decoder_bwd(packed, feat, layout, x, embed_pos, out, dout, saved, grads, M, precision: str = "f32", packed16=None,
                 wgrad_precision: str = "auto", recompute_h1: bool = False, return_tiles: bool = False,
-                deterministic: bool = False):
+                deterministic: bool = False, defer_reduce: Optional[dict] = None):
     if wgrad_precision == "auto":
         wgrad_precision = ("stream_" + precision) if (precision in SPLIT_PRECISIONS and embed_pos is None) else "f32"
     if getattr(saved, "mipsf_masks_only", False) and grads is not None:
@@ -431,15 +463,19 @@
                 raise RuntimeError("recompute_h1 needs wgrad_precision 'stream_f16x3' / 'stream_bf16x6' and packed16")
             if recompute_h1:
                 _check_family(packed16, wgrad_precision[len("stream_"):])
+            defer = defer_reduce is not None and live_list is not None and lean_dact and not deterministic
             a = _lib.DecoderWgrad16Args.new(live_list=dptr(live_list, torch.int32),
                                             M=M, packed16=dptr(packed16) if recompute_h1 else None, feat=dptr(feat), x=dptr(x),
                                             saved=dptr(saved), dact=dptr(dact), tile_live=dptr(tile_live, torch.int32),
                                             grads=C.pointer(st), partial=dptr(partial), feat_layout=layout, arithmetic=arith,
                                             flags=(_lib.WGRAD_LEAN_DACT if lean_dact else 0)
-                                            | (_lib.WGRAD_DETERMINISTIC if deterministic else 0),
+                                            | (_lib.WGRAD_DETERMINISTIC if deterministic else 0)
+                                            | (_lib.WGRAD_NO_REDUCE if defer else 0),
                                             packed16_floats=packed16.numel() if recompute_h1 else 0)
             with _timed("decoder_wgrad"):
                 check(lib().mipsf_decoder_wgrad16(C.byref(a), stream_ptr()), "decoder_wgrad16")
+            if defer:
+                defer_reduce.update(partial=partial, n_records=int(lib().mipsf_decoder_wgrad16_records(M)), grads=st)
             return (dfeat, dx, dpe, tiles) if return_tiles else (dfeat, dx, dpe)
         if recompute_h1:
             raise RuntimeError("recompute_h1 needs wgrad_precision 'stream_f16x3'")
```

After: 413.0 million rays*samples/s. 9.4% lower.
